# ruotianluo/ImageCaptioning.pytorch

Measured on NVIDIA H100. Metric: captions/sec at beam=5 seq_len=20, higher is better.
Workload: dtype f32 (fp32-grade: split-fp16 x3 tensor-core passes, fp32 accumulate)

## Files before the change

### imagecaptioning.pytorch_b200/_lib.py

```python
from __future__ import annotations

import ctypes
import os
from ctypes import POINTER, Structure, c_char_p, c_double, c_float, c_int, c_long, c_longlong, c_ulonglong, c_void_p

PKG = os.path.dirname(os.path.abspath(__file__))
LIB_PATH = os.path.join(PKG, 'libcapb200.so')

MODE_SIMT_FP32, MODE_TC_F16X3, MODE_TC_F16X1 = 0, 1, 2
MODES = {'simt_fp32': MODE_SIMT_FP32, 'tc_f16x3': MODE_TC_F16X3, 'tc_f16x1': MODE_TC_F16X1}
OP_MODES = dict(MODES, skinny_tf32x3=3, skinny_fp32=4, tf32x3_tc=5, tf32x3_tc_dgrad=6, tf32x3_tc_wgrad=7)
FAMILY_UPDOWN, FAMILY_NEWFC, FAMILY_ATT2IN2 = 0, 1, 2
FAMILY_AOA = 3
ENSEMBLE_MAX_MEMBERS = 8
SAMPLE_GREEDY, SAMPLE_MULTINOMIAL, SAMPLE_FORCED, SAMPLE_TEACHER, SAMPLE_TOPK, SAMPLE_TOPP = 0, 1, 2, 3, 4, 5


class ModelCfg(Structure):
    _fields_ = [('family', c_int), ('vocab_size', c_int), ('input_encoding_size', c_int), ('rnn_size', c_int), ('att_hid_size', c_int),
                ('fc_feat_size', c_int), ('att_feat_size', c_int), ('seq_length', c_int), ('numeric_mode', c_int)]


WEIGHT_FIELDS = ['embed', 'fc_embed_w', 'fc_embed_b', 'att_embed_w', 'att_embed_b', 'ctx2att_w', 'ctx2att_b', 'logit_w', 'logit_b',
                 'att_lstm_w_ih', 'att_lstm_w_hh', 'att_lstm_b_ih', 'att_lstm_b_hh', 'lang_lstm_w_ih', 'lang_lstm_w_hh', 'lang_lstm_b_ih',
# ... 183 lines not shown
    'capb200_vocab_select': (c_int, [c_void_p, c_long, c_int, c_int, c_int, c_float, c_float, c_ulonglong, c_ulonglong, c_void_p, c_int, c_void_p,
                                     c_void_p, c_void_p]),
    'capb200_engine_create': (c_void_p, [POINTER(ModelCfg)]),
    'capb200_engine_destroy': (None, [c_void_p]),
    'capb200_engine_bind_weights': (c_int, [c_void_p, POINTER(Weights), c_void_p]),
    'capb200_decode_beam': (c_int, [c_void_p, c_void_p, c_void_p, c_void_p, c_int, c_int, POINTER(BeamOpts), c_void_p, c_void_p, c_void_p, c_void_p,
                                    c_void_p, c_void_p, c_void_p]),
    'capb200_beam_record_logprobs': (c_int, [c_void_p, c_int, c_int, c_void_p, c_void_p]),
    'capb200_decode_beam_diverse': (c_int, [c_void_p, c_void_p, c_void_p, c_void_p, c_int, c_int, POINTER(DiverseOpts), c_void_p, c_void_p, c_void_p,
                                            c_void_p, c_void_p, c_void_p, c_void_p]),
    'capb200_decode_sample': (c_int, [c_void_p, c_void_p, c_void_p, c_void_p, c_int, c_int, POINTER(SampleOpts), c_void_p, c_long, c_void_p, c_void_p,
                                      c_void_p, c_void_p]),
    'capb200_engine_launch_count': (c_long, [c_void_p]),
    'capb200_engine_set_profiling': (c_int, [c_void_p, c_int]),
    'capb200_engine_read_profile': (c_int, [c_void_p, c_int, c_void_p, c_void_p, c_void_p, c_int]),
    'capb200_tfm_create': (c_void_p, [POINTER(TfmCfg)]),
    'capb200_tfm_destroy': (None, [c_void_p]),
    'capb200_tfm_bind_weights': (c_int, [c_void_p, POINTER(TfmWeights), c_void_p]),
    'capb200_tfm_decode_beam': (c_int, [c_void_p, c_void_p, c_void_p, c_int, c_int, POINTER(BeamOpts), c_void_p, c_void_p, c_void_p, c_void_p, c_void_p,
                                        c_void_p, c_void_p]),
    'capb200_tfm_beam_record_logprobs': (c_int, [c_void_p, c_int, c_int, c_void_p, c_void_p]),
    'capb200_tfm_decode_sample': (c_int, [c_void_p, c_void_p, c_void_p, c_int, c_int, POINTER(SampleOpts), c_void_p, c_long, c_void_p, c_void_p, c_void_p,
                                          c_void_p]),
    'capb200_tfm_launch_count': (c_long, [c_void_p]),
    'capb200_aoa_create': (c_void_p, [POINTER(AoaCfg)]),
    'capb200_aoa_destroy': (None, [c_void_p]),
    'capb200_aoa_bind_weights': (c_int, [c_void_p, POINTER(AoaWeights), c_void_p]),
    'capb200_aoa_decode_beam': (c_int, [c_void_p, c_void_p, c_void_p, c_int, c_int, POINTER(BeamOpts), c_void_p, c_void_p, c_void_p, c_void_p, c_void_p,
                                        c_void_p, c_void_p]),
    'capb200_aoa_beam_record_logprobs': (c_int, [c_void_p, c_int, c_int, c_void_p, c_void_p]),
    'capb200_aoa_decode_beam_diverse': (c_int, [c_void_p, c_void_p, c_void_p, c_int, c_int, POINTER(DiverseOpts), c_void_p, c_void_p, c_void_p, c_void_p,
                                                c_void_p, c_void_p, c_void_p]),
    'capb200_aoa_decode_sample': (c_int, [c_void_p, c_void_p, c_void_p, c_int, c_int, POINTER(SampleOpts), c_void_p, c_long, c_void_p, c_void_p, c_void_p,
                                          c_void_p]),
    'capb200_aoa_scst_step': (c_int, [c_void_p, c_void_p, c_int, c_int, POINTER(AoaScstOpts), c_void_p, c_void_p, c_void_p, c_int, POINTER(AoaWeights),
                                      c_void_p, c_void_p, c_void_p, c_void_p, c_void_p, c_void_p]),
    'capb200_aoa_xe_step': (c_int, [c_void_p, c_void_p, c_int, c_int, POINTER(AoaXeOpts), c_void_p, c_void_p, c_int, POINTER(AoaWeights), c_void_p,
                                    c_void_p, c_void_p]),
    'capb200_aoa_launch_count': (c_long, [c_void_p]),
    'capb200_ensemble_create': (c_void_p, []),
    'capb200_ensemble_destroy': (None, [c_void_p]),
    'capb200_ensemble_decode_beam': (c_int, [c_void_p, c_void_p, c_int, c_void_p, c_void_p, c_void_p, c_int, c_int, POINTER(BeamOpts), c_void_p, c_void_p,
                                             c_void_p, c_void_p, c_void_p, c_void_p, c_void_p]),
    'capb200_ensemble_beam_record_logprobs': (c_int, [c_void_p, c_int, c_int, c_void_p, c_void_p]),
    'capb200_ensemble_decode_sample': (c_int, [c_void_p, c_void_p, c_int, c_void_p, c_void_p, c_void_p, c_int, c_int, POINTER(SampleOpts), c_void_p, c_long,
                                               c_void_p, c_void_p, c_void_p, c_void_p]),
    'capb200_ensemble_launch_count': (c_long, [c_void_p]),
    'capb200_updown_scst_step': (c_int, [c_void_p, c_void_p, c_void_p, c_int, c_int, POINTER(ScstOpts), c_void_p, c_void_p, c_void_p, c_int,
                                         POINTER(UpdownGrads), c_void_p, c_void_p, c_void_p, c_void_p, c_void_p, c_void_p]),
    'capb200_att2in2_scst_step': (c_int, [c_void_p, c_void_p, c_void_p, c_int, c_int, POINTER(ScstOpts), c_void_p, c_void_p, c_void_p, c_int,
                                          POINTER(Att2in2Grads), c_void_p, c_void_p, c_void_p, c_void_p, c_void_p, c_void_p]),
    'capb200_att2in2_xe_step': (c_int, [c_void_p, c_void_p, c_void_p, c_int, c_int, POINTER(XeOpts), c_void_p, c_void_p, c_int, POINTER(Att2in2Grads),
                                        c_void_p, c_void_p, c_void_p]),
    'capb200_newfc_scst_step': (c_int, [c_void_p, c_void_p, c_void_p, c_int, c_int, POINTER(ScstOpts), c_void_p, c_void_p, c_void_p, c_int,
                                        POINTER(NewfcGrads), c_void_p, c_void_p, c_void_p, c_void_p, c_void_p, c_void_p]),
    'capb200_newfc_xe_step': (c_int, [c_void_p, c_void_p, c_void_p, c_int, c_int, POINTER(XeOpts), c_void_p, c_void_p, c_int, POINTER(NewfcGrads),
                                      c_void_p, c_void_p, c_void_p]),
    'capb200_dropout_mask': (c_int, [c_void_p, c_long, c_ulonglong, c_int, c_int, c_float, c_void_p]),
    'capb200_tfm_xe_step': (c_int, [c_void_p, c_void_p, c_int, c_int, POINTER(TfmXeOpts), c_void_p, c_void_p, c_int, POINTER(TfmWeights), c_void_p, c_void_p,
                                    c_void_p]),
    'capb200_tfm_scst_step': (c_int, [c_void_p, c_void_p, c_int, c_int, POINTER(TfmScstOpts), c_void_p, c_void_p, c_void_p, c_int, POINTER(TfmWeights),
                                      c_void_p, c_void_p, c_void_p, c_void_p, c_void_p, c_void_p]),
    'capb200_tfm_set_grad_events': (c_int, [c_void_p, c_void_p, c_int]),
    'capb200_adam_chunk_elems': (c_int, []),
    'capb200_adam_step': (c_int, [c_void_p, c_void_p, c_void_p, c_int, c_double, c_double, c_double, c_double, c_double, c_long, c_double, c_int, c_void_p]),
    'capb200_engine_set_grad_events': (c_int, [c_void_p, c_void_p, c_int]),
    'capb200_aoa_set_grad_events': (c_int, [c_void_p, c_void_p, c_int]),
    'capb200_cider_table_create': (c_void_p, [c_void_p, c_void_p, c_long, c_double, c_void_p]),
    'capb200_cider_table_destroy': (None, [c_void_p]),
    'capb200_cider_corpus_table_create': (c_void_p, []),
    'capb200_cider_table_reserve': (c_int, [c_void_p, c_long, c_int]),
    'capb200_cider_table_is_corpus': (c_int, [c_void_p]),
    'capb200_cider_scores': (c_int, [c_void_p, c_void_p, c_int, c_int, c_int, c_void_p, c_void_p, c_int, c_void_p, c_void_p, c_void_p]),
    'capb200_bleu4_scores': (c_int, [c_void_p, c_int, c_void_p, c_int, c_int, c_void_p, c_void_p, c_int, c_void_p, c_void_p]),
    'capb200_weighted_reward': (c_int, [c_void_p, POINTER(RewardWeights), c_void_p, c_int, c_void_p, c_int, c_int, c_void_p, c_void_p, c_int, c_void_p,
                                        c_void_p, c_void_p, c_void_p]),
    'capb200_updown_xe_step': (c_int, [c_void_p, c_void_p, c_void_p, c_int, c_int, POINTER(XeOpts), c_void_p, c_void_p, c_int, c_void_p, c_void_p,
                                       c_void_p, c_void_p]),
    'capb200_self_critical_reward': (c_int, [c_void_p, c_void_p, c_int, c_void_p, c_int, c_int, c_void_p, c_void_p, c_int, c_void_p, c_void_p,
                                             c_void_p]),
    'capb200_reward_criterion_forward': (c_int, [c_void_p, c_void_p, c_void_p, c_int, c_int, c_int, c_void_p, c_void_p, c_void_p, c_void_p]),
    'capb200_reward_criterion_backward': (c_int, [c_void_p, c_void_p, c_int, c_int, c_int, c_void_p, c_float, c_void_p, c_void_p]),
    'capb200_decode_gemm': (c_int, [c_void_p, c_void_p, c_int, c_int, c_int, c_int, POINTER(GemmEpilogue), c_void_p, c_int, c_void_p]),
    'capb200_updown_xe_vjp': (c_int, [c_void_p, c_void_p, c_void_p, c_int, c_int, POINTER(XeOpts), POINTER(VjpOpts), c_void_p, c_int,
                                      POINTER(UpdownGrads), c_void_p, c_void_p]),
    'capb200_updown_scst_vjp': (c_int, [c_void_p, c_void_p, c_void_p, c_int, c_int, POINTER(ScstOpts), POINTER(VjpOpts), POINTER(UpdownGrads),
                                        c_void_p, c_void_p, c_void_p]),
    'capb200_att2in2_xe_vjp': (c_int, [c_void_p, c_void_p, c_void_p, c_int, c_int, POINTER(XeOpts), POINTER(VjpOpts), c_void_p, c_int,
                                       POINTER(Att2in2Grads), c_void_p, c_void_p]),
    'capb200_att2in2_scst_vjp': (c_int, [c_void_p, c_void_p, c_void_p, c_int, c_int, POINTER(ScstOpts), POINTER(VjpOpts), POINTER(Att2in2Grads),
                                         c_void_p, c_void_p, c_void_p]),
    'capb200_newfc_xe_vjp': (c_int, [c_void_p, c_void_p, c_void_p, c_int, c_int, POINTER(XeOpts), POINTER(VjpOpts), c_void_p, c_int,
                                     POINTER(NewfcGrads), c_void_p, c_void_p]),
    'capb200_newfc_scst_vjp': (c_int, [c_void_p, c_void_p, c_void_p, c_int, c_int, POINTER(ScstOpts), POINTER(VjpOpts), POINTER(NewfcGrads),
                                       c_void_p, c_void_p, c_void_p]),
    'capb200_aoa_xe_vjp': (c_int, [c_void_p, c_void_p, c_int, c_int, POINTER(AoaXeOpts), POINTER(VjpOpts), c_void_p, c_int, POINTER(AoaWeights),
                                   c_void_p, c_void_p]),
    'capb200_aoa_scst_vjp': (c_int, [c_void_p, c_void_p, c_int, c_int, POINTER(AoaScstOpts), POINTER(VjpOpts), POINTER(AoaWeights), c_void_p,
                                     c_void_p, c_void_p]),
    'capb200_tfm_xe_vjp': (c_int, [c_void_p, c_void_p, c_int, c_int, POINTER(TfmXeOpts), POINTER(VjpOpts), c_void_p, c_int, POINTER(TfmWeights),
                                   c_void_p, c_void_p]),
    'capb200_tfm_scst_vjp': (c_int, [c_void_p, c_void_p, c_int, c_int, POINTER(TfmScstOpts), POINTER(VjpOpts), POINTER(TfmWeights), c_void_p,
                                     c_void_p, c_void_p]),
}

_lib = None


def load() -> ctypes.CDLL:
    global _lib
    if _lib is not None:
        return _lib
    if not os.path.exists(LIB_PATH):
        raise RuntimeError('capb200: %s is missing -- run `python imagecaptioning.pytorch_b200/build.py`; there is no CPU fallback' % LIB_PATH)
    lib = ctypes.CDLL(LIB_PATH)
    for name, (res, args) in SIGNATURES.items():
        fn = getattr(lib, name)
        fn.restype = res
        fn.argtypes = args
    if lib.capb200_abi_version() != 1:
        raise RuntimeError('capb200: ABI version mismatch')
    _lib = lib
    return lib


def check(rc: int, what: str = '') -> None:
    if rc != 0:
        msg = load().capb200_last_error()
        raise RuntimeError('capb200 %s failed: %s' % (what, msg.decode() if msg else 'unknown error'))


def ptr(t) -> int:
    if t is None:
        return None
    if hasattr(t, 'data_ptr'):
        return t.data_ptr()
    return t.ctypes.data


def current_stream() -> int:
    import torch
    return torch.cuda.current_stream().cuda_stream
```

### imagecaptioning.pytorch_b200/csrc/aoa_engine.cu

```cuda
#include <vector>

#include "../../include/capb200.h"
#include "common.cuh"
#include "engine_common.cuh"
#include "kernels.cuh"
#include "train_common.cuh"

using namespace capb200;

namespace capb200 {
__global__ void capb_add_vec_kernel(const float* a, const float* b, float* o, int n) {
    const int i = blockIdx.x * blockDim.x + threadIdx.x;
    if (i < n) o[i] = a[i] + b[i];
}
__global__ void capb_interleave_gates_kernel(const float* src, float* dst, int H) {
    const int i = blockIdx.x * blockDim.x + threadIdx.x;
    if (i < 4 * H) dst[i] = src[(i & 3) * H + (i >> 2)];
}
}

struct capb200_aoa_engine {
    capb200_aoa_cfg cfg{};
    capb200_aoa_weights w{};
    int V1 = 0, E = 0, H = 0, heads = 0, dk = 0, F = 0, T = 0, mode = 0;
// ... 11 lines not shown
    char* ws = nullptr;
    int capB = 0, capRows = 0, capR = 0, capBeam = 0;
    Planes in_att;
    Act rx, rln, rqkv, ratt, rt, att_e, mean, p_att_kv, g_mean;
    Act h0_in, h0_out, ctx_in, ctx_out, xt, gates, qln, qproj, att, t2;
    float* c0[2] = {nullptr, nullptr};
    long ld_c = 0;
    int core_cur = 0;
    DecodeBuffers d;
    std::vector<GemmTcPlan*> plans;
    char* tape = nullptr;
    size_t tape_bytes = 0;
    Tf32Context* tf32 = nullptr;
    cudaEvent_t grad_events[10] = {};
    cudaStream_t side = nullptr;
    cudaEvent_t ev_fork = nullptr, ev_join = nullptr;
    StepGraph sg;
};

namespace {

enum Site { A_ATT = 0, A_CTX, A_GMEAN, A_LSTM, A_Q, A_A2C, A_LOGIT, A_REF , A_COUNT = A_REF + 2 * CAPB200_AOA_REFINER_LAYERS };

void destroy_plans(capb200_aoa_engine* e) {
    for (auto& p : e->plans) { if (p) gemm_tc_plan_destroy(p); p = nullptr; }
}

int gemm(capb200_aoa_engine* e, int site, GemmProblem& g, int plan_rows, cudaStream_t st) {
    e->launches++;
    return run_gemm_mode(e->mode, &e->plans[site], g, plan_rows, st);
}

void layout_weights(capb200_aoa_engine* e, Arena& a) {
    const int H = e->H, E = e->E;
    for (int l = 0; l < CAPB200_AOA_REFINER_LAYERS; ++l) { e->r_qkv_w[l] = a.take<float>((long)3 * H * H); e->r_qkv_b[l] = a.take<float>(3 * H); }
    e->bsum = a.take<float>(4 * H);
    e->bsum_il = a.take<float>(4 * H);
    e->ld_xgate = round_up(4 * H, 8);
    e->xgate = a.take<float>((long)e->V1 * e->ld_xgate);
    if (!e->tc) return;
    e->p_att = carve_planes(a, H, e->F);
    e->p_ctx = carve_planes(a, 2 * H, H);
    e->p_logit = carve_planes(a, e->V1, H);
    e->p_ih_x = carve_planes(a, 4 * H, E);
    e->p_ih_c = carve_planes(a, 4 * H, H);
    e->p_hh = carve_planes(a, 4 * H, H);
    e->p_q = carve_planes(a, H, H);
    e->p_a2c_a = carve_planes(a, 2 * H, H);
    e->p_a2c_h = carve_planes(a, 2 * H, H);
    for (int l = 0; l < CAPB200_AOA_REFINER_LAYERS; ++l) {
        e->pr_qkv[l] = carve_planes(a, 3 * H, H);
        e->pr_aoa_a[l] = carve_planes(a, 2 * H, H);
        e->pr_aoa_q[l] = carve_planes(a, 2 * H, H);
    }
}

void layout_workspace(capb200_aoa_engine* e, Arena& a, int B, int rows, int R, int beam) {
    const int H = e->H, E = e->E, T = e->T;
    const bool tc = e->tc;
    const long BR = (long)B * R;
    if (tc) e->in_att = carve_planes(a, BR, e->F);
    e->rx.carve(a, BR, H, false);
    e->rln.carve(a, BR, H, tc);
    e->rqkv.carve(a, BR, 3 * H, false);
    e->ratt.carve(a, BR, H, tc);
    e->rt.carve(a, BR, 2 * H, false);
    e->att_e.carve(a, BR, H, tc);
    e->mean.carve(a, B, H, tc);
    e->p_att_kv.carve(a, BR, 2 * H, false);
    e->g_mean.carve(a, B, 4 * H, false);
    e->h0_in.carve(a, rows, H, tc);
    e->h0_out.carve(a, rows, H, tc);
    e->ctx_in.carve(a, rows, H, tc);
    e->ctx_out.carve(a, rows, H, tc);
    e->xt.carve(a, rows, E, tc);
    e->gates.carve(a, rows, 4 * H, false);
    e->qln.carve(a, rows, H, tc);
    e->qproj.carve(a, rows, H, false);
    e->att.carve(a, rows, H, tc);
    e->t2.carve(a, rows, 2 * H, false);
    e->ld_c = round_up(H, 8);
    for (int i = 0; i < 2; ++i) e->c0[i] = a.take<float>((long)rows * e->ld_c);
    e->d.carve(a, B, rows, beam, T);
}

int ensure_workspace(capb200_aoa_engine* e, int B, int rows, int R, int beam, cudaStream_t st) {
    if (B <= e->capB && rows <= e->capRows && R <= e->capR && beam <= e->capBeam && e->ws != nullptr) return 0;
    const int nB = B > e->capB ? B : e->capB, nRows = rows > e->capRows ? rows : e->capRows;
    const int nR = R > e->capR ? R : e->capR, nBeam = beam > e->capBeam ? beam : e->capBeam;
    Arena dry;
    layout_workspace(e, dry, nB, nRows, nR, nBeam);
    const size_t need = dry.off + 256;
    CAPB_CHECK_CUDA(cudaStreamSynchronize(st));
    destroy_plans(e);
    if (e->ws) CAPB_CHECK_CUDA(cudaFree(e->ws));
    e->ws = nullptr;
    CAPB_CHECK_CUDA(cudaMalloc(&e->ws, need));
    Arena real;
    real.base = e->ws;
    layout_workspace(e, real, nB, nRows, nR, nBeam);
    e->capB = nB; e->capRows = nRows; e->capR = nR; e->capBeam = nBeam;
    CAPB_CHECK_CUDA(cudaMemsetAsync(e->ws, 0, need, st));
    return fill_int_launch(e->d.neg1, nRows, -1, st);
}

int pack(capb200_aoa_engine* e, const float* w, long ldw, int rows, int cols, const Planes& p, cudaStream_t st) {
    e->launches++;
    return split_planes_launch(w, ldw, rows, cols, p.hi, p.lo, p.ld, st);
}
int pack_gates(capb200_aoa_engine* e, const float* w, long ldw, int H, int cols, const Planes& p, cudaStream_t st) {
    e->launches++;
    return split_planes_interleave_launch(w, ldw, H, cols, p.hi, p.lo, p.ld, st);
}

int prepare(capb200_aoa_engine* e, const float* att, const float* mask, int B, int R, cudaStream_t st) {
    CAPB_NVTX("capb200 aoa prepare_feature (att_embed, refiner, ctx2att)");
    const int H = e->H, E = e->E, BR = B * R, capBR = e->capB * e->capR;
    const capb200_aoa_weights& w = e->w;
    ActView in; in.f = const_cast<float*>(att); in.ld = e->F;
    if (e->tc) {
        e->launches++;
        if (split_planes_launch(att, e->F, BR, e->F, e->in_att.hi, e->in_att.lo, e->in_att.ld, st)) return 1;
        in.hi = e->in_att.hi; in.lo = e->in_att.lo;
    }
    {
        GemmProblem g;
        g.M = BR; g.N = H; g.nseg = 1;
        g.seg[0] = seg_of(in, w.att_embed_w, e->F, e->p_att, e->F);
        g.seg[0].lda_h = e->in_att.ld;
        g.epi.bias = w.att_embed_b; g.epi.relu = 1;
        g.epi.C = e->rx.v.f; g.epi.ldc = e->rx.v.ld;
        if (gemm(e, A_ATT, g, capBR, st)) return 1;
    }
    if (mask != nullptr) { e->launches++; if (mask_rows_launch(e->rx.v, B, R, H, mask, R, st)) return 1; }
    for (int l = 0; l < CAPB200_AOA_REFINER_LAYERS; ++l) {
        const capb200_aoa_refiner_layer& L = w.refiner[l];
        e->launches++;
        if (layer_norm_launch(BR, H, e->rx.v.f, e->rx.v.ld, L.ln_a, L.ln_b, 1e-6f, e->rln.v, st)) return 1;
        {
            GemmProblem g;
            g.M = BR; g.N = 3 * H; g.nseg = 1;
            g.seg[0] = seg_of(e->rln.v, e->r_qkv_w[l], H, e->pr_qkv[l], H);
            g.epi.bias = e->r_qkv_b[l];
            g.epi.C = e->rqkv.v.f; g.epi.ldc = e->rqkv.v.ld;
            if (gemm(e, A_REF + 2 * l, g, capBR, st)) return 1;
        }
        e->launches++;
        if (enc_self_attention_launch(B, R, e->heads, e->dk, e->rqkv.v.f, e->rqkv.v.f + H, e->rqkv.v.f + 2 * H, e->rqkv.v.ld, mask, R, e->ratt.v, st)) return 1;
        {
            GemmProblem g;
            g.M = BR; g.N = 2 * H; g.nseg = 2;
            g.seg[0] = seg_of(e->ratt.v, L.aoa_w, 2 * H, e->pr_aoa_a[l], H);
            g.seg[1] = seg_of(e->rln.v, L.aoa_w + H, 2 * H, e->pr_aoa_q[l], H);
            g.epi.bias = L.aoa_b;
            g.epi.C = e->rt.v.f; g.epi.ldc = e->rt.v.ld;
            if (gemm(e, A_REF + 2 * l + 1, g, capBR, st)) return 1;
        }
        e->launches++;
        ActView xo = e->rx.v;
        if (glu_launch(BR, H, e->rt.v.f, e->rt.v.ld, e->rx.v.f, e->rx.v.ld, xo, st)) return 1;
    }
    e->launches++;
    if (layer_norm_launch(BR, H, e->rx.v.f, e->rx.v.ld, w.refiner_norm_a, w.refiner_norm_b, 1e-6f, e->att_e.v, st)) return 1;
    e->launches++;
    if (masked_mean_launch(B, R, H, e->att_e.v.f, e->att_e.v.ld, mask, R, e->mean.v, st)) return 1;
    {
        GemmProblem g;
        g.M = BR; g.N = 2 * H; g.nseg = 1;
        g.seg[0] = seg_of(e->att_e.v, w.ctx2att_w, H, e->p_ctx, H);
        g.epi.bias = w.ctx2att_b;
        g.epi.C = e->p_att_kv.v.f; g.epi.ldc = e->p_att_kv.v.ld;
        if (gemm(e, A_CTX, g, capBR, st)) return 1;
    }
    {
        GemmProblem g;
        g.M = B; g.N = 4 * H; g.nseg = 1;
        g.seg[0] = seg_of(e->mean.v, w.att_lstm_w_ih + E, E + H, e->p_ih_c, H);
        g.epi.bias = e->tc ? e->bsum_il : e->bsum;
        g.epi.C = e->g_mean.v.f; g.epi.ldc = e->g_mean.v.ld;
        if (gemm(e, A_GMEAN, g, e->capB, st)) return 1;
    }
    return 0;
}

int core_step(capb200_aoa_engine* e, int rows, int rpi, const int* tokens, const int* src_row, float* logits, long ld_logits, int B, int R,
              const float* mask, cudaStream_t st) {
    const int H = e->H, E = e->E;
    const capb200_aoa_weights& w = e->w;
    StateCopy s0, s1;
    s0.src = e->h0_out.v.f; s0.ld_src = e->h0_out.v.ld; s0.dst = e->h0_in.v;
    s1.src = e->ctx_out.v.f; s1.ld_src = e->ctx_out.v.ld; s1.dst = e->ctx_in.v;
    e->launches++;
    if (state_gather_embed_launch(rows, tokens, src_row, w.embed, E, 0, 1, e->xt.v, H, 2, s0, s1, st)) return 1;
    const int cur = e->core_cur, nxt = cur ^ 1;
    {
        GemmProblem g;
        g.M = rows; g.N = 4 * H; g.nseg = 2;
        g.seg[0] = seg_of(e->ctx_in.v, w.att_lstm_w_ih + E, E + H, e->p_ih_c, H);
        g.seg[1] = seg_of(e->h0_in.v, w.att_lstm_w_hh, H, e->p_hh, H);
        g.epi.row_bias = e->g_mean.v.f; g.epi.ld_row_bias = e->g_mean.v.ld; g.epi.rows_per_group = rpi;
        if (e->tc) {
            g.epi.lstm = 1; g.epi.H = H;
            g.epi.c_prev = e->c0[cur]; g.epi.ld_cprev = e->ld_c; g.epi.src_row = src_row;
            g.epi.c_out = e->c0[nxt]; g.epi.ld_cout = e->ld_c;
            g.epi.gather_bias = e->xgate; g.epi.ld_gb = e->ld_xgate; g.epi.gather_idx = tokens;
            g.epi.h_f = e->h0_out.v.f; g.epi.h_hi = e->h0_out.v.hi; g.epi.h_lo = e->h0_out.v.lo; g.epi.ld_h = e->h0_out.v.ld;
        } else {
            g.epi.C = e->gates.v.f; g.epi.ldc = e->gates.v.ld;
        }
        if (gemm(e, A_LSTM, g, e->capRows, st)) return 1;
    }
    if (!e->tc) {
        e->launches++;
        if (lstm_pointwise_launch(rows, H, e->gates.v.f, e->gates.v.ld, src_row, e->c0[cur], e->ld_c, e->c0[nxt], e->ld_c, e->h0_out.v, e->xgate,
                                  e->ld_xgate, tokens, st)) return 1;
    }
    e->core_cur = nxt;
    e->launches++;
    if (layer_norm_launch(rows, H, e->h0_out.v.f, e->h0_out.v.ld, w.attn_norm_a, w.attn_norm_b, 1e-6f, e->qln.v, st)) return 1;
    {
        GemmProblem g;
        g.M = rows; g.N = H; g.nseg = 1;
        g.seg[0] = seg_of(e->qln.v, w.attn_q_w, H, e->p_q, H);
        g.epi.bias = w.attn_q_b;
        g.epi.C = e->qproj.v.f; g.epi.ldc = e->qproj.v.ld;
        if (gemm(e, A_Q, g, e->capRows, st)) return 1;
    }
    e->launches++;
    if (cross_attention_launch(rows, rpi, e->heads, e->dk, R, e->qproj.v.f, e->qproj.v.ld, e->p_att_kv.v.f + H, e->p_att_kv.v.f, e->p_att_kv.v.ld, mask, R,
                               e->att.v, st)) return 1;
    {
        GemmProblem g;
        g.M = rows; g.N = 2 * H; g.nseg = 2;
        g.seg[0] = seg_of(e->att.v, w.att2ctx_w, 2 * H, e->p_a2c_a, H);
        g.seg[1] = seg_of(e->h0_out.v, w.att2ctx_w + H, 2 * H, e->p_a2c_h, H);
        g.epi.bias = w.att2ctx_b;
        g.epi.C = e->t2.v.f; g.epi.ldc = e->t2.v.ld;
        if (gemm(e, A_A2C, g, e->capRows, st)) return 1;
    }
    e->launches++;
    if (glu_launch(rows, H, e->t2.v.f, e->t2.v.ld, nullptr, 0, e->ctx_out.v, st)) return 1;
    GemmProblem g;
    g.M = rows; g.N = e->V1; g.nseg = 1;
    g.seg[0] = seg_of(e->ctx_out.v, w.logit_w, H, e->p_logit, H);
    g.epi.bias = w.logit_b;
    g.epi.C = logits; g.epi.ldc = ld_logits;
    (void)B;
    return gemm(e, A_LOGIT, g, e->capRows, st);
}

int check_ready(capb200_aoa_engine* e) {
    CAPB_REQUIRE(e != nullptr, "null engine");
    CAPB_REQUIRE(e->bound, "capb200_aoa_bind_weights has not been called");
    CAPB_CHECK_RANGE();
    return 0;
}

}

namespace capb200 {

int aoa_member_info(capb200_aoa_engine* e, MemberInfo* m) {
    if (check_ready(e)) return 1;
    m->family = CAPB200_FAMILY_AOA;
    m->V1 = e->V1; m->T = e->T;
    m->attends = true;
    m->graph_ok = true;
    m->ws = e->ws; m->wblock = e->wblock;
    m->fresh = e->d.neg1;
    m->launches = &e->launches;
    return 0;
}

int aoa_decode_workspace(capb200_aoa_engine* e, int B, int rows, int R, int beam, cudaStream_t st) {
    return ensure_workspace(e, B, rows, R, beam, st);
}

int aoa_decode_prepare(capb200_aoa_engine* e, const float* att, const float* mask, int B, int R, cudaStream_t st) {
    if (prepare(e, att, mask, B, R, st)) return 1;
    e->core_cur = 0;
    return 0;
}

int aoa_decode_core(capb200_aoa_engine* e, int rows, int rpi, const int* tokens, const int* src_row, float* logits, long ld, int R,
                    const float* mask, cudaStream_t st) {
    return core_step(e, rows, rpi, tokens, src_row, logits, ld, 0, R, mask, st);
}

}

extern "C" {

capb200_aoa_engine* capb200_aoa_create(const capb200_aoa_cfg* c) {
    if (c == nullptr) { set_error("null cfg"); return nullptr; }
    if (c->heads < 1 || c->rnn_size % c->heads != 0) { set_error("rnn_size must be divisible by the head count"); return nullptr; }
    if (c->numeric_mode < 0 || c->numeric_mode > 2) { set_error("unknown numeric mode"); return nullptr; }
    if (c->seq_length < 1 || c->seq_length > 64) { set_error("seq_length must be in 1..64"); return nullptr; }
    int ndev = 0;
    if (cudaGetDeviceCount(&ndev) != cudaSuccess || ndev == 0) { set_error("no CUDA device: the capb200 engine has no CPU fallback"); return nullptr; }
    capb200_aoa_engine* e = new capb200_aoa_engine();
    e->cfg = *c;
    e->V1 = c->vocab_size + 1; e->E = c->input_encoding_size; e->H = c->rnn_size; e->heads = c->heads; e->dk = c->rnn_size / c->heads;
    e->F = c->att_feat_size; e->T = c->seq_length; e->mode = c->numeric_mode;
    e->tc = c->numeric_mode != CAPB200_MODE_SIMT_FP32;
    e->plans.assign(A_COUNT, nullptr);
    return e;
}

void capb200_aoa_destroy(capb200_aoa_engine* e) {
    if (e == nullptr) return;
    destroy_plans(e);
    cudaFree(e->wblock);
    cudaFree(e->ws);
    e->d.release();
    cudaFree(e->tape);
    e->sg.destroy();
    tf32_context_destroy(e->tf32);
    if (e->ev_fork) cudaEventDestroy(e->ev_fork);
    if (e->ev_join) cudaEventDestroy(e->ev_join);
    if (e->side) cudaStreamDestroy(e->side);
    delete e;
}

long capb200_aoa_launch_count(const capb200_aoa_engine* e) { return e ? e->launches : 0; }

int capb200_aoa_bind_weights(capb200_aoa_engine* e, const capb200_aoa_weights* w, void* stream) {
    CAPB_REQUIRE(e != nullptr && w != nullptr, "null argument");
    cudaStream_t st = static_cast<cudaStream_t>(stream);
    CAPB_REQUIRE(w->embed && w->att_embed_w && w->ctx2att_w && w->att_lstm_w_ih && w->att_lstm_w_hh && w->attn_q_w && w->att2ctx_w && w->logit_w,
// ... 429 lines not shown
```

### imagecaptioning.pytorch_b200/csrc/common.cuh

```cuda
#pragma once
#include <atomic>
#include <cstdint>
#include <cstdio>
#include <cstring>
#include <string>
#include <cuda.h>
#include <cuda_fp16.h>
#include <cuda_runtime.h>

namespace capb200 {

void set_error(const std::string& msg);
#define CAPB_CHECK_CUDA(expr)                                                                          \
    do {                                                                                               \
        cudaError_t _e = (expr);                                                                       \
        if (_e != cudaSuccess) {                                                                       \
            capb200::set_error(std::string(#expr) + " failed: " + cudaGetErrorString(_e) + " at " +    \
                               __FILE__ + ":" + std::to_string(__LINE__));                            \
            return 1;                                                                                  \
        }                                                                                              \
    } while (0)
#define CAPB_REQUIRE(cond, msg)                                                                        \
    do {                                                                                               \
        if (!(cond)) {                                                                                 \
            capb200::set_error(std::string("requirement failed: ") + #cond + " -- " + (msg));          \
            return 1;                                                                                  \
        }                                                                                              \
    } while (0)

inline int cdiv(int a, int b) { return (a + b - 1) / b; }
inline long round_up(long a, long b) { return (a + b - 1) / b * b; }

inline bool first_use_on_device(std::atomic<unsigned long long>& mask) {
    int dev = 0;
    if (cudaGetDevice(&dev) != cudaSuccess || dev < 0 || dev > 63) return true;
    const unsigned long long bit = 1ull << dev;
    return (mask.fetch_or(bit) & bit) == 0;
}

inline int sm_count() {
    static std::atomic<int> cache[64];
    int dev = 0;
    if (cudaGetDevice(&dev) != cudaSuccess || dev < 0 || dev > 63) dev = 0;
    int n = cache[dev].load();
    if (n == 0) {
        if (cudaDeviceGetAttribute(&n, cudaDevAttrMultiProcessorCount, dev) != cudaSuccess || n < 1) n = 132;
        cache[dev].store(n);
    }
    return n;
}

__device__ __forceinline__ void split_f32(float x, __half& hi, __half& lo) {
    hi = __float2half_rn(x);
    lo = __float2half_rn(x - __half2float(hi));
}

constexpr int kMaxSeg = 3;
struct GemmSeg {
    const float* A = nullptr;
    long lda = 0;
    const float* W = nullptr;
    long ldw = 0;
    const __half* A_hi = nullptr;
    const __half* A_lo = nullptr;
    long lda_h = 0;
    const __half* W_hi = nullptr;
    const __half* W_lo = nullptr;
    long ldw_h = 0;
    int K = 0;
};
struct GemmEpilogue {
    const float* bias = nullptr;
    const float* row_bias = nullptr;
    long ld_row_bias = 0;
    int rows_per_group = 1;
    const float* residual = nullptr;
    long ld_res = 0;
    int relu = 0;
    float* C = nullptr;
    long ldc = 0;
    __half* C_hi = nullptr;
    __half* C_lo = nullptr;
    long ldcs = 0;
    int lstm = 0;
    int H = 0;
    const float* c_prev = nullptr;
    long ld_cprev = 0;
    const int* src_row = nullptr;
    float* c_out = nullptr;
    long ld_cout = 0;
    const float* gather_bias = nullptr;
    long ld_gb = 0;
    const int* gather_idx = nullptr;
    float* h_f = nullptr;
    __half* h_hi = nullptr;
    __half* h_lo = nullptr;
    long ld_h = 0;
    unsigned long long* trace = nullptr;
};

__device__ __forceinline__ float fast_sigmoid(float x) { return __fdividef(1.0f, 1.0f + __expf(-x)); }
__device__ __forceinline__ float fast_tanh(float x) {
    const float e = __expf(2.0f * x);
    return 1.0f - __fdividef(2.0f, 1.0f + e);
}
__device__ __forceinline__ void fast_tanh4(const float (&x)[4], float (&t)[4]) {
    float y[4];
#pragma unroll
    for (int i = 0; i < 4; ++i) y[i] = 1.0f + __expf(fminf(2.0f * x[i], 20.0f));
    const float p01 = y[0] * y[1], p23 = y[2] * y[3];
    const float r = __fdividef(1.0f, p01 * p23);
    const float r01 = r * p23, r23 = r * p01;
    t[0] = fmaf(-2.0f, r01 * y[1], 1.0f);
    t[1] = fmaf(-2.0f, r01 * y[0], 1.0f);
    t[2] = fmaf(-2.0f, r23 * y[3], 1.0f);
    t[3] = fmaf(-2.0f, r23 * y[2], 1.0f);
}
struct GemmProblem {
    int M = 0, N = 0, nseg = 0;
    GemmSeg seg[kMaxSeg];
    GemmEpilogue epi;
};

enum NumericMode : int {
    kModeSimtFp32 = 0,
    kModeTcF16x3 = 1,
    kModeTcF16x1 = 2,
};

int gemm_simt_launch(const GemmProblem& p, cudaStream_t stream);

struct GemmTcPlan;
GemmTcPlan* gemm_tc_plan_create(const GemmProblem& p, int passes);
int gemm_tc_tile_n(int M, int N);
int gemm_tc_tile_m(int M, int N, int bn);
void gemm_tc_plan_destroy(GemmTcPlan* plan);
int gemm_tc_plan_launch(GemmTcPlan* plan, const GemmEpilogue* epi_override, int M_override, cudaStream_t stream);
bool gemm_tc_supported(const GemmProblem& p, std::string* why);

int split_planes_launch(const float* x, long ldx, int rows, int cols, __half* hi, __half* lo, long ldh, cudaStream_t stream);
int* range_flag_ptr();
int range_flag_read(int reset);
#define CAPB_CHECK_RANGE()                                                                                              \
    do {                                                                                                                \
        if (capb200::range_flag_read(0)) {                                                                              \
            capb200::set_error("a value with |x| >= 65504 (or inf/nan) reached a split-fp16 conversion in an earlier call: results of the "   \
                               "tensor-core modes are invalid for such inputs/weights (DESIGN.md section 3); capb200_range_status(1) clears the flag"); \
            return 1;                                                                                                   \
        }                                                                                                               \
    } while (0)
int split_planes_interleave_launch(const float* x, long ldx, int H, int cols, __half* hi, __half* lo, long ldh, cudaStream_t stream);

}
```

### imagecaptioning.pytorch_b200/csrc/engine.cu

```cuda
#include <map>
#include <mutex>
#include <vector>

#include "../../include/capb200.h"
#include "common.cuh"
#include "kernels.cuh"
#include "engine_common.cuh"
#include "train_common.cuh"

namespace capb200 {

static thread_local std::string g_last_error;
void set_error(const std::string& msg) { g_last_error = msg; }
const char* last_error_cstr() { return g_last_error.c_str(); }

__global__ void capb_fill_int_kernel(int* p, int n, int v) {
    const int i = blockIdx.x * blockDim.x + threadIdx.x;
    if (i < n) p[i] = v;
}
__global__ void capb_load_token_column_kernel(const long long* src, long ld, int col, int n, int* dst) {
    const int i = blockIdx.x * blockDim.x + threadIdx.x;
    if (i < n) dst[i] = (int)src[(long)i * ld + col];
}
__global__ void capb_store_token_column_kernel(const int* src, int n, long long* dst, long ld, int col) {
// ... 104 lines not shown
}

void layout_weights(capb200_engine* e, Arena& a) {
    const int H = e->H, E = e->E, A = e->A, V1 = e->V1;
    const bool updown = e->cfg.family == CAPB200_FAMILY_UPDOWN;
    e->bsum_att = a.take<float>(4 * H);
    e->bsum_lang = a.take<float>(4 * H);
    e->bsum_core = a.take<float>(5 * H);
    e->bsum_att_il = a.take<float>(4 * H);
    e->bsum_lang_il = a.take<float>(4 * H);
    if (updown) { e->ld_xgate = round_up(4 * H, 8); e->xgate = a.take<float>((long)V1 * e->ld_xgate); }
    if (!e->tc) return;
    e->p_logit = carve_planes(a, V1, H);
    if (updown) {
        e->p_fc = carve_planes(a, H, e->cfg.fc_feat_size);
        e->p_attw = carve_planes(a, H, e->cfg.att_feat_size);
        e->p_ctx = carve_planes(a, A, H);
        e->p_a_ih_h = carve_planes(a, 4 * H, H);
        e->p_a_ih_fc = carve_planes(a, 4 * H, H);
        e->p_a_ih_x = carve_planes(a, 4 * H, E);
        e->p_a_hh = carve_planes(a, 4 * H, H);
        e->p_l_ih_a = carve_planes(a, 4 * H, H);
        e->p_l_ih_h = carve_planes(a, 4 * H, H);
        e->p_l_hh = carve_planes(a, 4 * H, H);
        e->p_h2att = carve_planes(a, A, H);
    } else if (e->cfg.family == CAPB200_FAMILY_ATT2IN2) {
        e->p_attw = carve_planes(a, H, e->cfg.att_feat_size);
        e->p_ctx = carve_planes(a, A, H);
        e->p_h2att = carve_planes(a, A, H);
        e->p_i2h = carve_planes(a, 5 * H, E);
        e->p_h2h = carve_planes(a, 5 * H, H);
        e->p_a2c = carve_planes(a, 2 * H, H);
    } else {
        e->p_fc = carve_planes(a, E, e->cfg.fc_feat_size);
        e->p_i2h = carve_planes(a, 5 * H, E);
        e->p_h2h = carve_planes(a, 5 * H, H);
    }
}

bool attends(const capb200_engine* e) { return e->cfg.family != CAPB200_FAMILY_NEWFC; }

int pack(capb200_engine* e, const float* w, long ldw, int rows, int cols, const Planes& p, cudaStream_t st) {
    e->launches++;
    return split_planes_launch(w, ldw, rows, cols, p.hi, p.lo, p.ld, st);
}
int pack_gates(capb200_engine* e, const float* w, long ldw, int H, int cols, const Planes& p, cudaStream_t st) {
    e->launches++;
    return split_planes_interleave_launch(w, ldw, H, cols, p.hi, p.lo, p.ld, st);
}

void layout_workspace(capb200_engine* e, Arena& a, int B, int rows, int R, int beam) {
    const int H = e->H, E = e->E, A = e->A, T = e->T;
    const bool updown = e->cfg.family == CAPB200_FAMILY_UPDOWN;
    const bool attn = attends(e);
    const bool tc = e->tc;
    if (tc) {
        e->in_fc = carve_planes(a, B, e->cfg.fc_feat_size);
        if (attn) e->in_att = carve_planes(a, (long)B * R, e->cfg.att_feat_size);
    }
    e->fc_e.carve(a, B, updown ? H : E, tc);
    if (attn) {
        e->att_e.carve(a, (long)B * R, H, tc);
        e->p_att.carve(a, (long)B * R, A, false);
        e->att_res.carve(a, rows, H, tc);
        e->att_h.carve(a, rows, A, false);
    }
    if (updown) {
        e->g_fc.carve(a, B, 4 * H, false);
        e->h1_in.carve(a, rows, H, tc);
        e->h1_out.carve(a, rows, H, tc);
    }
    e->xt.carve(a, rows, E, tc);
    e->h0_in.carve(a, rows, H, tc);
    e->h0_out.carve(a, rows, H, tc);
    e->gates.carve(a, rows, 5 * H, false);
    e->ld_c = round_up(H, 8);
    for (int i = 0; i < 2; ++i) {
        e->c0[i] = a.take<float>((long)rows * e->ld_c);
        e->c1[i] = a.take<float>((long)rows * e->ld_c);
    }
    e->img_of_row = a.take<int>(rows);
    e->att_score = a.take<float>((long)rows * (R > 0 ? R : 1));
    e->d.carve(a, B, rows, beam, T);
}

int ensure_workspace(capb200_engine* e, int B, int rows, int R, int beam, cudaStream_t st) {
    if (B <= e->capB && rows <= e->capRows && R <= e->capR && beam <= e->capBeam && e->ws != nullptr) return 0;
    const int nB = B > e->capB ? B : e->capB, nRows = rows > e->capRows ? rows : e->capRows;
    const int nR = R > e->capR ? R : e->capR, nBeam = beam > e->capBeam ? beam : e->capBeam;
    Arena dry;
    layout_workspace(e, dry, nB, nRows, nR, nBeam);
    const size_t need = dry.off + 256;
    CAPB_CHECK_CUDA(cudaStreamSynchronize(st));
    destroy_plans(e);
    if (e->ws) CAPB_CHECK_CUDA(cudaFree(e->ws));
    e->ws = nullptr;
    CAPB_CHECK_CUDA(cudaMalloc(&e->ws, need));
    e->ws_bytes = need;
    Arena real;
    real.base = e->ws;
    layout_workspace(e, real, nB, nRows, nR, nBeam);
    e->capB = nB; e->capRows = nRows; e->capR = nR; e->capBeam = nBeam;
    CAPB_CHECK_CUDA(cudaMemsetAsync(e->ws, 0, need, st));
    return fill_int_launch(e->d.neg1, nRows, -1, st);
}

int run_gemm_inner(capb200_engine* e, int id, GemmProblem& g, int plan_rows, cudaStream_t st) {
    e->launches++;
    if (!e->tc) return gemm_simt_launch(g, st);
    if (e->plans[id] == nullptr) {
        GemmProblem planned = g;
        planned.M = plan_rows;
        e->plans[id] = gemm_tc_plan_create(planned, e->mode == CAPB200_MODE_TC_F16X3 ? 3 : 1);
        if (e->plans[id] == nullptr) return 1;
    }
    return gemm_tc_plan_launch(e->plans[id], &g.epi, g.M, st);
}

int run_gemm(capb200_engine* e, int id, GemmProblem& g, int plan_rows, cudaStream_t st) {
    if (!e->profiling) return run_gemm_inner(e, id, g, plan_rows, st);
    if (e->ev_used + 2 > e->ev_pool.size()) {
        for (int i = 0; i < 64; ++i) {
            cudaEvent_t ev;
            CAPB_CHECK_CUDA(cudaEventCreate(&ev));
            e->ev_pool.push_back(ev);
        }
    }
    double k_total = 0;
    for (int s = 0; s < g.nseg; ++s) k_total += g.seg[s].K;
    CAPB_CHECK_CUDA(cudaEventRecord(e->ev_pool[e->ev_used], st));
    const int rc = run_gemm_inner(e, id, g, plan_rows, st);
    CAPB_CHECK_CUDA(cudaEventRecord(e->ev_pool[e->ev_used + 1], st));
    e->ev_used += 2;
    e->ev_ids.push_back(id);
    e->ev_flops.push_back(2.0 * g.M * g.N * k_total);
    return rc;
}

int prepare(capb200_engine* e, const float* fc, const float* att, const float* mask, int B, int R, cudaStream_t st) {
    CAPB_NVTX("capb200 prepare_feature (fc_embed, att_embed, ctx2att)");
    const int H = e->H, E = e->E, A = e->A;
    const bool updown = e->cfg.family == CAPB200_FAMILY_UPDOWN;
    const capb200_weights& w = e->w;
    ActView fc_in;  fc_in.f = const_cast<float*>(fc);  fc_in.ld = e->cfg.fc_feat_size;
    if (e->tc && e->cfg.family != CAPB200_FAMILY_ATT2IN2) {
        e->launches++;
        if (split_planes_launch(fc, e->cfg.fc_feat_size, B, e->cfg.fc_feat_size, e->in_fc.hi, e->in_fc.lo, e->in_fc.ld, st)) return 1;
    }
    if (e->cfg.family != CAPB200_FAMILY_ATT2IN2) {
        GemmProblem g;
        g.M = B; g.N = updown ? H : E; g.nseg = 1;
        g.seg[0] = seg_of(fc_in, w.fc_embed_w, e->cfg.fc_feat_size, e->p_fc, e->cfg.fc_feat_size);
        g.seg[0].A_hi = e->in_fc.hi; g.seg[0].A_lo = e->in_fc.lo; g.seg[0].lda_h = e->in_fc.ld;
        g.epi.bias = w.fc_embed_b; g.epi.relu = updown ? 1 : 0;
        g.epi.C = e->fc_e.v.f; g.epi.ldc = e->fc_e.v.ld; g.epi.C_hi = e->fc_e.v.hi; g.epi.C_lo = e->fc_e.v.lo; g.epi.ldcs = e->fc_e.v.ld;
        if (run_gemm(e, G_FC, g, e->capB, st)) return 1;
    }
    if (!attends(e)) return 0;
    ActView att_in; att_in.f = const_cast<float*>(att); att_in.ld = e->cfg.att_feat_size;
    if (e->tc) {
        e->launches++;
        if (split_planes_launch(att, e->cfg.att_feat_size, B * R, e->cfg.att_feat_size, e->in_att.hi, e->in_att.lo, e->in_att.ld, st)) return 1;
    }
    {
        GemmProblem g;
        g.M = B * R; g.N = H; g.nseg = 1;
// ... 24 lines not shown
        g.epi.C = e->g_fc.v.f; g.epi.ldc = e->g_fc.v.ld;
        if (run_gemm(e, G_GFC, g, e->capB, st)) return 1;
    }
    return 0;
}

int core_step(capb200_engine* e, int rows, int rpi, const int* tokens, const int* src_row, float* logits, long ld_logits, int n_images, int R,
              const float* mask, cudaStream_t st) {
    const int H = e->H, E = e->E, A = e->A, V1 = e->V1;
    const capb200_weights& w = e->w;
    if (e->cfg.family == CAPB200_FAMILY_UPDOWN) {
        StateCopy s0, s1;
        s0.src = e->h0_out.v.f; s0.ld_src = e->h0_out.v.ld; s0.dst = e->h0_in.v;
        s1.src = e->h1_out.v.f; s1.ld_src = e->h1_out.v.ld; s1.dst = e->h1_in.v;
        const bool xg = e->use_xgate;
        e->launches++;
        if (state_gather_embed_launch(rows, tokens, src_row, w.embed, E, xg ? 0 : E, 1, e->xt.v, H, 2, s0, s1, st)) return 1;
        const int cur = e->core_cur, nxt = cur ^ 1;
        {
            GemmProblem g;
            g.M = rows; g.N = 4 * H;
            g.seg[0] = seg_of(e->h1_in.v, w.att_lstm_w_ih, E + 2 * H, e->p_a_ih_h, H);
            g.seg[1] = seg_of(e->h0_in.v, w.att_lstm_w_hh, H, e->p_a_hh, H);
            g.nseg = 2;
            if (!xg) { g.seg[2] = seg_of(e->xt.v, w.att_lstm_w_ih + 2 * H, E + 2 * H, e->p_a_ih_x, E); g.nseg = 3; }
            g.epi.row_bias = e->g_fc.v.f; g.epi.ld_row_bias = e->g_fc.v.ld; g.epi.rows_per_group = rpi;
            if (e->tc) {
                g.epi.lstm = 1; g.epi.H = H;
                g.epi.c_prev = e->c0[cur]; g.epi.ld_cprev = e->ld_c; g.epi.src_row = src_row;
                g.epi.c_out = e->c0[nxt]; g.epi.ld_cout = e->ld_c;
                g.epi.gather_bias = xg ? e->xgate : nullptr; g.epi.ld_gb = e->ld_xgate; g.epi.gather_idx = tokens;
                g.epi.h_f = e->h0_out.v.f; g.epi.h_hi = e->h0_out.v.hi; g.epi.h_lo = e->h0_out.v.lo; g.epi.ld_h = e->h0_out.v.ld;
            } else {
                g.epi.C = e->gates.v.f; g.epi.ldc = e->gates.v.ld;
            }
            if (run_gemm(e, G_LSTM1, g, e->capRows, st)) return 1;
        }
        if (!e->tc) {
            e->launches++;
            if (lstm_pointwise_launch(rows, H, e->gates.v.f, e->gates.v.ld, src_row, e->c0[cur], e->ld_c, e->c0[nxt], e->ld_c, e->h0_out.v,
                                      xg ? e->xgate : nullptr, e->ld_xgate, tokens, st)) return 1;
        }
        {
            GemmProblem g;
            g.M = rows; g.N = A; g.nseg = 1;
            g.seg[0] = seg_of(e->h0_out.v, w.h2att_w, H, e->p_h2att, H);
            g.epi.bias = w.h2att_b;
            g.epi.C = e->att_h.v.f; g.epi.ldc = e->att_h.v.ld;
            if (run_gemm(e, G_H2ATT, g, e->capRows, st)) return 1;
        }
        e->launches += 2;
        if (additive_attention_launch(n_images, rpi, R, A, H, e->att_h.v.f, e->att_h.v.ld, e->p_att.v.f, e->p_att.v.ld, e->att_e.v.f, e->att_e.v.ld,
                                      mask, R, w.alpha_w, w.alpha_b, e->att_score, e->att_res.v, st)) return 1;
        {
            GemmProblem g;
            g.M = rows; g.N = 4 * H; g.nseg = 3;
            g.seg[0] = seg_of(e->att_res.v, w.lang_lstm_w_ih, 2 * H, e->p_l_ih_a, H);
            g.seg[1] = seg_of(e->h0_out.v, w.lang_lstm_w_ih + H, 2 * H, e->p_l_ih_h, H);
            g.seg[2] = seg_of(e->h1_in.v, w.lang_lstm_w_hh, H, e->p_l_hh, H);
            if (e->tc) {
                g.epi.bias = e->bsum_lang_il;
                g.epi.lstm = 1; g.epi.H = H;
                g.epi.c_prev = e->c1[cur]; g.epi.ld_cprev = e->ld_c; g.epi.src_row = src_row;
                g.epi.c_out = e->c1[nxt]; g.epi.ld_cout = e->ld_c;
                g.epi.h_f = e->h1_out.v.f; g.epi.h_hi = e->h1_out.v.hi; g.epi.h_lo = e->h1_out.v.lo; g.epi.ld_h = e->h1_out.v.ld;
            } else {
                g.epi.bias = e->bsum_lang;
                g.epi.C = e->gates.v.f; g.epi.ldc = e->gates.v.ld;
            }
            if (run_gemm(e, G_LSTM2, g, e->capRows, st)) return 1;
        }
        if (!e->tc) {
            e->launches++;
            if (lstm_pointwise_launch(rows, H, e->gates.v.f, e->gates.v.ld, src_row, e->c1[cur], e->ld_c, e->c1[nxt], e->ld_c, e->h1_out.v,
                                      nullptr, 0, nullptr, st)) return 1;
        }
        e->core_cur = nxt;
        {
            GemmProblem g;
            g.M = rows; g.N = V1; g.nseg = 1;
            g.seg[0] = seg_of(e->h1_out.v, w.logit_w, H, e->p_logit, H);
            g.epi.bias = w.logit_b;
            g.epi.C = logits; g.epi.ldc = ld_logits;
            if (run_gemm(e, G_LOGIT, g, e->capRows, st)) return 1;
        }
        return 0;
    }
    if (e->cfg.family == CAPB200_FAMILY_ATT2IN2) {
        StateCopy s0, s1;
        s0.src = e->h0_out.v.f; s0.ld_src = e->h0_out.v.ld; s0.dst = e->h0_in.v;
        e->launches++;
        if (state_gather_embed_launch(rows, tokens, src_row, w.embed, E, E, 1, e->xt.v, H, 1, s0, s1, st)) return 1;
        const int cur = e->core_cur, nxt = cur ^ 1;
        {
            GemmProblem g;
            g.M = rows; g.N = A; g.nseg = 1;
            g.seg[0] = seg_of(e->h0_in.v, w.h2att_w, H, e->p_h2att, H);
            g.epi.bias = w.h2att_b;
            g.epi.C = e->att_h.v.f; g.epi.ldc = e->att_h.v.ld;
            if (run_gemm(e, G_H2ATT, g, e->capRows, st)) return 1;
        }
        e->launches += 2;
        if (additive_attention_launch(n_images, rpi, R, A, H, e->att_h.v.f, e->att_h.v.ld, e->p_att.v.f, e->p_att.v.ld, e->att_e.v.f, e->att_e.v.ld,
                                      mask, R, w.alpha_w, w.alpha_b, e->att_score, e->att_res.v, st)) return 1;
        {
            GemmProblem g;
            g.M = rows; g.N = 5 * H; g.nseg = 2;
            g.seg[0] = seg_of(e->xt.v, w.i2h_w, E, e->p_i2h, E);
            g.seg[1] = seg_of(e->h0_in.v, w.h2h_w, H, e->p_h2h, H);
            g.epi.bias = e->bsum_core;
            g.epi.C = e->gates.v.f; g.epi.ldc = e->gates.v.ld;
            if (run_gemm(e, G_CORE, g, e->capRows, st)) return 1;
        }
        {
            GemmProblem g;
            g.M = rows; g.N = 2 * H; g.nseg = 1;
            g.seg[0] = seg_of(e->att_res.v, w.a2c_w, H, e->p_a2c, H);
            g.epi.residual = e->gates.v.f + 3 * H; g.epi.ld_res = e->gates.v.ld;
            g.epi.C = e->gates.v.f + 3 * H; g.epi.ldc = e->gates.v.ld;
            if (run_gemm(e, G_A2C, g, e->capRows, st)) return 1;
        }
        e->launches++;
        if (maxout_pointwise_launch(rows, H, e->gates.v.f, e->gates.v.ld, src_row, e->c0[cur], e->ld_c, e->c0[nxt], e->ld_c, e->h0_out.v, st)) return 1;
        e->core_cur = nxt;
        GemmProblem g;
        g.M = rows; g.N = V1; g.nseg = 1;
        g.seg[0] = seg_of(e->h0_out.v, w.logit_w, H, e->p_logit, H);
        g.epi.bias = w.logit_b;
        g.epi.C = logits; g.epi.ldc = ld_logits;
        return run_gemm(e, G_LOGIT, g, e->capRows, st);
    }
    const bool fresh = (src_row == e->d.neg1);
    for (int pass = fresh ? 0 : 1; pass < 2; ++pass) {
        StateCopy s0, s1;
        s0.src = e->h0_out.v.f; s0.ld_src = e->h0_out.v.ld; s0.dst = e->h0_in.v;
        const int* srcs = (pass == 0) ? e->d.neg1 : (fresh ? nullptr : src_row);
        e->launches++;
        if (pass == 0) {
            if (state_gather_embed_launch(rows, e->img_of_row, srcs, e->fc_e.v.f, e->fc_e.v.ld, E, 0, e->xt.v, H, 1, s0, s1, st)) return 1;
        } else {
            if (state_gather_embed_launch(rows, tokens, srcs, w.embed, E, E, 0, e->xt.v, H, 1, s0, s1, st)) return 1;
        }
        const int cur = e->core_cur, nxt = cur ^ 1;
        GemmProblem g;
        g.M = rows; g.N = 5 * H; g.nseg = 2;
        g.seg[0] = seg_of(e->xt.v, w.i2h_w, E, e->p_i2h, E);
        g.seg[1] = seg_of(e->h0_in.v, w.h2h_w, H, e->p_h2h, H);
        g.epi.bias = e->bsum_core;
        g.epi.C = e->gates.v.f; g.epi.ldc = e->gates.v.ld;
        if (run_gemm(e, G_CORE, g, e->capRows, st)) return 1;
        e->launches++;
        if (maxout_pointwise_launch(rows, H, e->gates.v.f, e->gates.v.ld, srcs, e->c0[cur], e->ld_c, e->c0[nxt], e->ld_c, e->h0_out.v, st)) return 1;
        e->core_cur = nxt;
    }
    GemmProblem g;
    g.M = rows; g.N = V1; g.nseg = 1;
    g.seg[0] = seg_of(e->h0_out.v, w.logit_w, H, e->p_logit, H);
    g.epi.bias = w.logit_b;
    g.epi.C = logits; g.epi.ldc = ld_logits;
    return run_gemm(e, G_LOGIT, g, e->capRows, st);
}

int check_ready(capb200_engine* e) {
    CAPB_REQUIRE(e != nullptr, "null engine");
    CAPB_REQUIRE(e->bound, "capb200_engine_bind_weights has not been called");
    CAPB_CHECK_RANGE();
    return 0;
}

}

namespace capb200 {

int lstm_member_info(capb200_engine* e, MemberInfo* m) {
    if (check_ready(e)) return 1;
    m->family = e->cfg.family;
    m->V1 = e->V1; m->T = e->T;
    m->attends = attends(e);
    m->graph_ok = !e->profiling;
    m->ws = e->ws; m->wblock = e->wblock;
    m->fresh = e->d.neg1;
    m->launches = &e->launches;
    return 0;
}

int lstm_decode_workspace(capb200_engine* e, int B, int rows, int R, int beam, int rows_per_image, cudaStream_t st) {
    if (ensure_workspace(e, B, rows, R, beam, st)) return 1;
    if (!attends(e)) { iota_div_kernel<<<cdiv(rows, 256), 256, 0, st>>>(e->img_of_row, rows, rows_per_image); e->launches++; }
    return 0;
}

int lstm_decode_prepare(capb200_engine* e, const float* fc, const float* att, const float* mask, int B, int R, cudaStream_t st) {
    if (prepare(e, fc, att, mask, B, R, st)) return 1;
    e->core_cur = 0;
    return 0;
}

int lstm_decode_core(capb200_engine* e, int rows, int rpi, const int* tokens, const int* src_row, float* logits, long ld, int B, int R,
                     const float* mask, cudaStream_t st) {
    return core_step(e, rows, rpi, tokens, src_row, logits, ld, B, R, mask, st);
}

}

extern "C" {

const char* capb200_last_error(void) { return g_last_error.c_str(); }
int capb200_abi_version(void) { return CAPB200_ABI_VERSION; }
int capb200_range_status(int reset) { return range_flag_read(reset); }

capb200_engine* capb200_engine_create(const capb200_model_cfg* cfg) {
    if (cfg == nullptr) { set_error("null cfg"); return nullptr; }
    if (cfg->family != CAPB200_FAMILY_UPDOWN && cfg->family != CAPB200_FAMILY_NEWFC && cfg->family != CAPB200_FAMILY_ATT2IN2) {
        set_error("unknown model family");
        return nullptr;
    }
    if (cfg->numeric_mode < 0 || cfg->numeric_mode > 2) { set_error("unknown numeric mode"); return nullptr; }
    if (cfg->seq_length < 1 || cfg->seq_length > 64) { set_error("seq_length must be in 1..64"); return nullptr; }
    int ndev = 0;
    if (cudaGetDeviceCount(&ndev) != cudaSuccess || ndev == 0) {
        set_error("no CUDA device: the capb200 engine has no CPU fallback");
        return nullptr;
    }
    capb200_engine* e = new capb200_engine();
    e->cfg = *cfg;
    e->V1 = cfg->vocab_size + 1;
    e->E = cfg->input_encoding_size;
    e->H = cfg->rnn_size;
    e->A = cfg->att_hid_size;
    e->T = cfg->seq_length;
    e->mode = cfg->numeric_mode;
    e->tc = cfg->numeric_mode != CAPB200_MODE_SIMT_FP32;
    return e;
}

void capb200_engine_destroy(capb200_engine* e) {
    if (e == nullptr) return;
    destroy_plans(e);
    for (cudaEvent_t ev : e->ev_pool) cudaEventDestroy(ev);
    cudaFree(e->wblock);
    cudaFree(e->ws);
    e->d.release();
// ... 324 lines not shown
    g.seg[0].A = x; g.seg[0].lda = K; g.seg[0].W = w; g.seg[0].ldw = K; g.seg[0].K = K;
    g.epi.bias = b; g.epi.C = y; g.epi.ldc = N;
    const long ldh = round_up(K, 64);
    __half* scratch = nullptr;
    GemmTcPlan* plan = nullptr;
    int rc = 0;
    if (mode != CAPB200_MODE_SIMT_FP32) {
        CAPB_CHECK_CUDA(cudaMalloc(&scratch, (size_t)(M + N) * ldh * 2 * sizeof(__half)));
        __half* xh = scratch; __half* xl = xh + (size_t)M * ldh;
        __half* wh = xl + (size_t)M * ldh; __half* wl = wh + (size_t)N * ldh;
        rc = split_planes_launch(x, K, M, K, xh, xl, ldh, st) | split_planes_launch(w, K, N, K, wh, wl, ldh, st);
        g.seg[0].A_hi = xh; g.seg[0].A_lo = xl; g.seg[0].lda_h = ldh;
        g.seg[0].W_hi = wh; g.seg[0].W_lo = wl; g.seg[0].ldw_h = ldh;
        plan = rc ? nullptr : gemm_tc_plan_create(g, mode == CAPB200_MODE_TC_F16X3 ? 3 : 1);
        if (plan == nullptr) rc = 1;
    }
    cudaEvent_t e0, e1;
    cudaEventCreate(&e0);
    cudaEventCreate(&e1);
    for (int i = 0; i < 3 + iters && !rc; ++i) {
        if (i == 3) cudaEventRecord(e0, st);
        rc = plan ? gemm_tc_plan_launch(plan, nullptr, 0, st) : gemm_simt_launch(g, st);
    }
    cudaEventRecord(e1, st);
    if (cudaStreamSynchronize(st) != cudaSuccess) { set_error(std::string("bench_linear: ") + cudaGetErrorString(cudaGetLastError())); rc = 1; }
    float ms = 0.f;
    if (!rc) { cudaEventElapsedTime(&ms, e0, e1); *ms_per_launch = ms / iters; }
    cudaEventDestroy(e0);
    cudaEventDestroy(e1);
    if (plan) gemm_tc_plan_destroy(plan);
    if (scratch) cudaFree(scratch);
    return rc;
}

int capb200_decode_gemm(const float* x, const float* w, int M, int N, int K, int mode, const capb200_gemm_epilogue* epi, unsigned long long* trace_host,
                        int n_slots, void* stream) {
    cudaStream_t st = static_cast<cudaStream_t>(stream);
    CAPB_REQUIRE(x && w && epi && M > 0 && N > 0 && K > 0, "bad argument");
    CAPB_REQUIRE(mode == CAPB200_MODE_TC_F16X3 || mode == CAPB200_MODE_TC_F16X1, "the decode GEMM runs in the tc_f16x3 / tc_f16x1 modes");
    CAPB_REQUIRE(trace_host == nullptr || (n_slots >= 296 * 16 && mode == CAPB200_MODE_TC_F16X3), "the trace needs 296 x 16 slots and tc_f16x3");
    GemmProblem g;
    g.M = M; g.N = N; g.nseg = 1;
    g.seg[0].K = K;
    GemmEpilogue& e = g.epi;
    e.bias = epi->bias; e.row_bias = epi->row_bias; e.ld_row_bias = epi->ld_row_bias; e.rows_per_group = epi->rows_per_group;
    e.residual = epi->residual; e.ld_res = epi->ld_res; e.relu = epi->relu;
    e.C = epi->C; e.ldc = epi->ldc;
    e.C_hi = reinterpret_cast<__half*>(epi->C_hi); e.C_lo = reinterpret_cast<__half*>(epi->C_lo); e.ldcs = epi->ldcs;
    e.lstm = epi->lstm; e.H = epi->H;
    e.c_prev = epi->c_prev; e.ld_cprev = epi->ld_cprev; e.src_row = epi->src_row;
    e.c_out = epi->c_out; e.ld_cout = epi->ld_cout;
    e.gather_bias = epi->gather_bias; e.ld_gb = epi->ld_gb; e.gather_idx = epi->gather_idx;
    e.h_f = epi->h_f; e.h_hi = reinterpret_cast<__half*>(epi->h_hi); e.h_lo = reinterpret_cast<__half*>(epi->h_lo); e.ld_h = epi->ld_h;
    CAPB_REQUIRE(e.C_hi == nullptr || e.C_lo != nullptr, "C_hi needs C_lo");
    CAPB_REQUIRE(e.h_hi == nullptr || e.h_lo != nullptr, "h_hi needs h_lo");
    CAPB_REQUIRE(e.row_bias == nullptr || e.rows_per_group >= 1, "rows_per_group must be >= 1");
    CAPB_REQUIRE(e.gather_bias == nullptr || e.gather_idx != nullptr, "gather_bias needs gather_idx");
    const long ldh = round_up(K, 64);
    __half* scratch = nullptr;
    unsigned long long* trace = nullptr;
    CAPB_CHECK_CUDA(cudaMalloc(&scratch, (size_t)(M + N) * ldh * 2 * sizeof(__half)));
    if (trace_host != nullptr) {
        CAPB_CHECK_CUDA(cudaMalloc(&trace, sizeof(unsigned long long) * 296 * 16));
        CAPB_CHECK_CUDA(cudaMemsetAsync(trace, 0, sizeof(unsigned long long) * 296 * 16, st));
    }
    __half* xh = scratch; __half* xl = xh + (size_t)M * ldh;
    __half* wh = xl + (size_t)M * ldh; __half* wl = wh + (size_t)N * ldh;
    int rc = split_planes_launch(x, K, M, K, xh, xl, ldh, st) | split_planes_launch(w, K, N, K, wh, wl, ldh, st);
    g.seg[0].A_hi = xh; g.seg[0].A_lo = xl; g.seg[0].lda_h = ldh;
    g.seg[0].W_hi = wh; g.seg[0].W_lo = wl; g.seg[0].ldw_h = ldh;
    GemmTcPlan* plan = rc ? nullptr : gemm_tc_plan_create(g, mode == CAPB200_MODE_TC_F16X3 ? 3 : 1);
    if (plan == nullptr) rc = 1;
    for (int i = 0; i < (trace ? 3 : 1) && !rc; ++i) rc = gemm_tc_plan_launch(plan, nullptr, 0, st);
    if (!rc && trace) {
        GemmEpilogue ep = g.epi;
        ep.trace = trace;
        rc = gemm_tc_plan_launch(plan, &ep, 0, st);
    }
    if (cudaStreamSynchronize(st) != cudaSuccess) { set_error(std::string("decode_gemm: ") + cudaGetErrorString(cudaGetLastError())); rc = 1; }
    if (!rc && trace) CAPB_CHECK_CUDA(cudaMemcpy(trace_host, trace, sizeof(unsigned long long) * 296 * 16, cudaMemcpyDeviceToHost));
    if (plan) gemm_tc_plan_destroy(plan);
    cudaFree(scratch);
    if (trace) cudaFree(trace);
    return rc;
}

int capb200_gemm_tile_n(int M, int N) { return gemm_tc_tile_n(M, N); }

int capb200_gemm_tile_m(int M, int N) { return gemm_tc_tile_m(M, N, gemm_tc_tile_n(M, N)); }

int capb200_lstm_cell(const float* x, int Kx, const float* h, const float* c, const float* w_ih, const float* w_hh, const float* b_ih,
                      const float* b_hh, float* h_out, float* c_out, int M, int H, int mode, void* stream) {
    cudaStream_t st = static_cast<cudaStream_t>(stream);
    CAPB_REQUIRE(x && h && c && w_ih && w_hh && b_ih && b_hh && h_out && c_out, "null argument");
    float* gates = nullptr;
    CAPB_CHECK_CUDA(cudaMallocAsync(&gates, sizeof(float) * ((size_t)M * 4 * H + 4 * H), st));
    float* bsum = gates + (size_t)M * 4 * H;
    add_vec_kernel<<<cdiv(4 * H, 256), 256, 0, st>>>(b_ih, b_hh, bsum, 4 * H);
    int rc = capb200_linear(x, Kx, w_ih, Kx, bsum, gates, 4 * H, M, 4 * H, Kx, 0, mode, stream);
    float* g2 = nullptr;
    if (!rc) {
        CAPB_CHECK_CUDA(cudaMallocAsync(&g2, sizeof(float) * (size_t)M * 4 * H, st));
        rc = capb200_linear(h, H, w_hh, H, nullptr, g2, 4 * H, M, 4 * H, H, 0, mode, stream);
        if (!rc) add_vec_kernel<<<cdiv(M * 4 * H, 256), 256, 0, st>>>(gates, g2, gates, M * 4 * H);
    }
    if (!rc) {
        ActView ho; ho.f = h_out; ho.ld = H;
        rc = lstm_pointwise_launch(M, H, gates, 4 * H, nullptr, c, H, c_out, H, ho, nullptr, 0, nullptr, st);
    }
    if (g2) cudaFreeAsync(g2, st);
    cudaFreeAsync(gates, st);
    return rc;
}

int capb200_additive_attention(const float* att_h, const float* p_att, const float* att, const float* mask, const float* alpha_w,
                               const float* alpha_b, float* out, int n_images, int rows_per_image, int R, int A, int H, void* stream) {
    CAPB_REQUIRE(att_h && p_att && att && alpha_w && alpha_b && out, "null argument");
    ActView o; o.f = out; o.ld = H;
    cudaStream_t st = static_cast<cudaStream_t>(stream);
    float* scratch = nullptr;
    CAPB_CHECK_CUDA(cudaMallocAsync(&scratch, sizeof(float) * (size_t)n_images * rows_per_image * R, st));
    const int rc = additive_attention_launch(n_images, rows_per_image, R, A, H, att_h, A, p_att, A, att, H, mask, R, alpha_w, alpha_b, scratch, o, st);
    cudaFreeAsync(scratch, st);
    return rc;
}

int capb200_log_softmax_topk(float* logits, long ld, int rows, int V1, int twice, int k, float* top_val, int* top_idx, void* stream) {
    CAPB_REQUIRE(logits != nullptr && rows > 0 && V1 > 0, "bad argument");
    VocabStepArgs va;
    va.rows = rows; va.V1 = V1; va.logits = logits; va.ld = ld; va.twice = twice; va.topk = k; va.top_val = top_val; va.top_idx = top_idx;
    return vocab_step_launch(va, static_cast<cudaStream_t>(stream));
}

int capb200_vocab_stats_topk(const float* logits, long ld, int rows, int V1, int twice, int k, float* stats, float* top_val, int* top_idx, void* stream) {
    CAPB_REQUIRE(logits != nullptr && stats != nullptr && top_val != nullptr && top_idx != nullptr, "null argument");
    CAPB_REQUIRE(rows > 0 && V1 > 0 && ld >= V1 && k > 0, "bad argument");
    CAPB_REQUIRE((reinterpret_cast<uintptr_t>(stats) & 7) == 0, "stats must be 8-byte aligned");
    VocabStepArgs va;
    va.rows = rows; va.V1 = V1; va.logits = const_cast<float*>(logits); va.ld = ld; va.twice = twice;
    va.topk = k; va.top_val = top_val; va.top_idx = top_idx;
    va.stats = reinterpret_cast<float2*>(stats);
    return vocab_step_launch(va, static_cast<cudaStream_t>(stream));
}

int capb200_vocab_select(float* logits, long ld, int rows, int V1, int select, float top, float temperature, unsigned long long seed,
                         unsigned long long step, int* unfinished, int first_step, int* tokens_out, float* picked_lp, void* stream) {
    CAPB_REQUIRE(logits != nullptr && tokens_out != nullptr && picked_lp != nullptr, "null argument");
    CAPB_REQUIRE(rows > 0 && V1 > 0 && ld >= V1, "bad argument");
    CAPB_REQUIRE(select == 1 || select == 2 || select == 4 || select == 5, "select must be 1 (greedy), 2 (multinomial), 4 (top-k) or 5 (nucleus)");
    CAPB_REQUIRE(temperature > 0.f, "temperature must be positive");
    CAPB_REQUIRE(select != 4 || top >= 1.f, "top-k sampling needs k >= 1");
    CAPB_REQUIRE(select != 5 || (top > 0.f && top <= 1.f), "nucleus sampling needs 0 < p <= 1");
    VocabStepArgs va;
    va.rows = rows; va.V1 = V1; va.logits = logits; va.ld = ld;
    va.select = select; va.top = top; va.temperature = temperature; va.seed = seed; va.step = step;
    va.unfinished = unfinished; va.first_step = first_step; va.tokens_out = tokens_out; va.picked_lp = picked_lp;
    return vocab_step_launch(va, static_cast<cudaStream_t>(stream));
}

}

namespace {

struct Tape : StepTape {
    int* tok;
    float *xt, *g1, *h0, *c0, *atth, *alpha, *attres, *g2, *h1, *c1, *out;
// ... 679 lines not shown
```

### imagecaptioning.pytorch_b200/csrc/engine_common.cuh

```cuda
#pragma once
#include <cstdio>
#include <cstdlib>
#include <cstring>

#include "../../include/capb200.h"
#include "common.cuh"
#include "kernels.cuh"
#include "nvtx.cuh"

struct capb200_cider_table {
    capb200::CiderTable* t = nullptr;
};

namespace capb200 {

struct Planes {
    __half* hi = nullptr;
    __half* lo = nullptr;
    long ld = 0;
};

struct Arena {
    char* base = nullptr;
    size_t off = 0;
    template <typename T>
    T* take(size_t n) {
        off = (off + 255) & ~size_t(255);
        T* p = base ? reinterpret_cast<T*>(base + off) : nullptr;
        off += n * sizeof(T);
        return p;
    }
};

struct Act {
    ActView v;
    void carve(Arena& a, long rows, long cols, bool planes) {
        v.ld = round_up(cols, 64);
        v.f = a.take<float>(rows * v.ld);
        if (planes) {
            v.hi = a.take<__half>(rows * v.ld);
            v.lo = a.take<__half>(rows * v.ld);
        } else {
            v.hi = v.lo = nullptr;
        }
    }
};

inline DecodeEdits to_edits(const capb200_decode_edits& c) {
    DecodeEdits e;
    e.constraint = c.decoding_constraint;
    e.unk_col = c.unk_col;
    e.n_bad = (c.bad_endings != nullptr && c.n_bad_endings > 0) ? c.n_bad_endings : 0;
    e.bad = c.bad_endings;
    e.trigrams = c.block_trigrams;
    e.trigram_rows = c.trigram_rows;
    return e;
}

inline Planes carve_planes(Arena& a, long rows, long cols) {
    Planes p;
    p.ld = round_up(cols, 64);
    p.hi = a.take<__half>(rows * p.ld);
    p.lo = a.take<__half>(rows * p.ld);
    return p;
}


inline GemmSeg seg_of(const ActView& a, const float* w, long ldw, const Planes& wp, int K) {
    GemmSeg s;
    s.A = a.f; s.lda = a.ld; s.W = w; s.ldw = ldw;
    s.A_hi = a.hi; s.A_lo = a.lo; s.lda_h = a.ld;
    s.W_hi = wp.hi; s.W_lo = wp.lo; s.ldw_h = wp.ld;
    s.K = K;
    return s;
}


inline int run_gemm_mode(int mode, GemmTcPlan** plan, GemmProblem& g, int plan_rows, cudaStream_t st) {
    if (mode == 0) return gemm_simt_launch(g, st);
    if (*plan == nullptr) {
        GemmProblem planned = g;
        planned.M = plan_rows;
        *plan = gemm_tc_plan_create(planned, mode == 1 ? 3 : 1);
        if (*plan == nullptr) return 1;
    }
    return gemm_tc_plan_launch(*plan, &g.epi, g.M, st);
}


struct DecodeBuffers {
    int *tokens = nullptr, *src_row = nullptr, *neg1 = nullptr, *unfinished = nullptr, *forced = nullptr;
    float* top_val = nullptr;
    int* top_idx = nullptr;
    float* top_val_e = nullptr;
    int* top_idx_e = nullptr;
    float2* slab_stats = nullptr;
    BeamState bs;
    long long* rec_seq = nullptr;
    int *rec_len = nullptr, *rec_hist = nullptr, *out_hist = nullptr, *tmp_len = nullptr;
    float *rec_p = nullptr, *rec_raw = nullptr, *tmp_p = nullptr, *tmp_raw = nullptr;
    float* slab = nullptr;
    size_t slab_bytes = 0;
    float2* dbs_stats = nullptr;
    size_t dbs_stats_bytes = 0;
    int* dbs_done_cnt = nullptr;
    size_t dbs_done_bytes = 0;
    const float2* last_stats = nullptr;
    long slab_step_stride = 0;
    int last_B = 0, last_beam = 0;
    DecodeEdits last_edits;
    cudaGraphExec_t loop_exec = nullptr;
    unsigned long long loop_key[8] = {0, 0, 0, 0, 0, 0, 0, 0}, seen_key[8] = {0, 0, 0, 0, 0, 0, 0, 0};
    long loop_launches = 0;
    bool graph_broken = false;

    void release() {
        if (loop_exec) cudaGraphExecDestroy(loop_exec);
        loop_exec = nullptr;
        cudaFree(slab);
        cudaFree(dbs_stats);
        cudaFree(dbs_done_cnt);
        slab = nullptr; dbs_stats = nullptr; dbs_done_cnt = nullptr;
    }

    void carve(Arena& a, int B, int rows, int beam, int T) {
        tokens = a.take<int>(rows);
        src_row = a.take<int>(rows);
        neg1 = a.take<int>(rows);
        unfinished = a.take<int>(rows);
        forced = a.take<int>(rows);
        top_val = a.take<float>((long)rows * 16);
        top_idx = a.take<int>((long)rows * 16);
        top_val_e = a.take<float>((long)rows * 16);
        top_idx_e = a.take<int>((long)rows * 16);
        slab_stats = a.take<float2>((long)rows * T);
        const long rec = (long)B * beam * T;
        bs.sums = a.take<float>((long)B * beam);
        bs.seq_a = a.take<int>(rec);
        bs.seq_b = a.take<int>(rec);
        bs.hist_a = a.take<int>(rec);
        bs.hist_b = a.take<int>(rec);
        bs.done_cnt = a.take<int>(B);
        bs.done_seq = a.take<int>(rec * T);
        bs.done_hist = a.take<int>(rec * T);
        bs.done_len = a.take<int>(rec);
        bs.done_p = a.take<double>(rec);
        bs.done_raw = a.take<float>(rec);
        bs.tokens = tokens;
        bs.src_row = src_row;
        rec_seq = a.take<long long>(rec);
        rec_hist = a.take<int>(rec);
        out_hist = a.take<int>(rec);
        rec_len = a.take<int>((long)B * beam);
        rec_p = a.take<float>((long)B * beam);
        rec_raw = a.take<float>((long)B * beam);
        tmp_len = a.take<int>((long)B * beam);
        tmp_p = a.take<float>((long)B * beam);
        tmp_raw = a.take<float>((long)B * beam);
    }
};

__global__ void capb_fill_int_kernel(int* p, int n, int v);
__global__ void capb_load_token_column_kernel(const long long* src, long ld, int col, int n, int* dst);
int fill_int_launch(int* p, int n, int v, cudaStream_t st);
int load_token_column_launch(const long long* src, long ld, int col, int n, int* dst, cudaStream_t st);
int store_token_column_launch(const int* src, int n, long long* dst, long ld, int col, cudaStream_t st);

inline const int* beam_ancestors(const BeamState& s, int t) { return ((t - 1) & 1) ? s.hist_a : s.hist_b; }

inline unsigned long long loop_graph_key(const void* ws, const void* wblock, const void* mask, int R, int family) {
    unsigned long long h = 1469598103934665603ull;
    auto mix = [&](unsigned long long v) { h ^= v; h *= 1099511628211ull; };
    mix(reinterpret_cast<uintptr_t>(ws)); mix(reinterpret_cast<uintptr_t>(wblock)); mix(reinterpret_cast<uintptr_t>(mask));
    mix((unsigned long long)R); mix((unsigned long long)family + 17);
    return h | 1ull;
}

inline int grow_buffer(void** p, size_t* bytes, size_t need, cudaStream_t st) {
    if (need <= *bytes) return 0;
    CAPB_CHECK_CUDA(cudaStreamSynchronize(st));
    if (*p) CAPB_CHECK_CUDA(cudaFree(*p));
    *p = nullptr;
    *bytes = 0;
    const cudaError_t e = cudaMalloc(p, need);
    if (e != cudaSuccess) {
        (void)cudaGetLastError();
        *p = nullptr;
        set_error("cannot allocate " + std::to_string(need >> 20) + " MB of device workspace (" + cudaGetErrorString(e) +
                  "); its size grows with batch, length and V + 1: DESIGN.md, 'Vocabularies above 51 199 words'");
        return 1;
    }
    *bytes = need;
    return 0;
}

template <class Loop>
int run_beam_loop(DecodeBuffers& d, const unsigned long long (&key)[8], bool use_graph, long* launches, cudaStream_t st, Loop run_loop) {
    static const bool graphs_off = getenv("CAPB200_NO_GRAPH") != nullptr;
    const bool debug = getenv("CAPB200_GRAPH_DEBUG") != nullptr;
    const bool try_graph = use_graph && !graphs_off && !d.graph_broken;
    if (try_graph && d.loop_exec != nullptr && memcmp(key, d.loop_key, sizeof(key)) == 0) {
        CAPB_CHECK_CUDA(cudaGraphLaunch(d.loop_exec, st));
        *launches += d.loop_launches;
        if (debug) fprintf(stderr, "capb200: beam loop replayed from its CUDA graph\n");
    } else if (try_graph && memcmp(key, d.seen_key, sizeof(key)) == 0) {
        if (d.loop_exec != nullptr) { cudaGraphExecDestroy(d.loop_exec); d.loop_exec = nullptr; }
        const long l0 = *launches;
        cudaGraph_t graph = nullptr;
        bool ok = cudaStreamBeginCapture(st, cudaStreamCaptureModeThreadLocal) == cudaSuccess;
        const int rc = ok ? run_loop() : 1;
        if (ok) ok = cudaStreamEndCapture(st, &graph) == cudaSuccess && graph != nullptr && rc == 0;
        if (ok) ok = cudaGraphInstantiate(&d.loop_exec, graph, 0) == cudaSuccess;
        if (graph != nullptr) cudaGraphDestroy(graph);
        if (!ok) {
            (void)cudaGetLastError();
            d.loop_exec = nullptr;
            d.graph_broken = true;
            *launches = l0;
            if (run_loop()) return 1;
        } else {
            d.loop_launches = *launches - l0;
            memcpy(d.loop_key, key, sizeof(key));
            CAPB_CHECK_CUDA(cudaGraphLaunch(d.loop_exec, st));
            if (debug) fprintf(stderr, "capb200: beam loop captured into a CUDA graph (%ld launches)\n", d.loop_launches);
        }
    } else {
        memcpy(d.seen_key, key, sizeof(key));
        if (run_loop()) return 1;
    }
    return 0;
}

template <class CoreFn>
int beam_decode_driver(DecodeBuffers& d, int V1, int T, int B, int beam, int keep, int penalty_kind, float penalty_alpha, long long* seq,
                       float* seq_logprobs, long long* done_seq, int* done_len, float* done_p, float* done_raw, CoreFn core, long* launches,
                       cudaStream_t st, unsigned long long graph_key = 0, const DecodeEdits& ed = DecodeEdits(), float temperature = 1.0f) {
    const int rows = B * beam;
    const bool edits = ed.any();
    const int k_in = beam + ed.kinds();
    CAPB_REQUIRE(!ed.trigrams, "block_trigrams applies to _sample only (AttModel.py:306)");
    CAPB_REQUIRE(k_in <= 16, "beam_size + number of active decode edits (decoding_constraint, remove_bad_endings, UNK suppression) must be <= 16");
    if (temperature == 0.f) temperature = 1.0f;
    CAPB_REQUIRE(temperature > 0.f, "temperature must be positive");
    if (grow_buffer(reinterpret_cast<void**>(&d.slab), &d.slab_bytes, (size_t)T * rows * V1 * sizeof(float), st)) return 1;
    d.slab_step_stride = (long)rows * V1;
    d.last_B = B;
    d.last_beam = beam;
    BeamState s = d.bs;
    s.B = B; s.beam = beam; s.T = T; s.V1 = V1;
    auto run_loop = [&]() -> int {
        CAPB_NVTX("capb200 beam loop (T steps: core, vocab stats, beam step)");
        CAPB_CHECK_CUDA(cudaMemsetAsync(s.sums, 0, sizeof(float) * B * beam, st));
        CAPB_CHECK_CUDA(cudaMemsetAsync(s.done_cnt, 0, sizeof(int) * B, st));
        CAPB_CHECK_CUDA(cudaMemsetAsync(d.tokens, 0, sizeof(int) * rows, st));
        for (int t = 0; t < T; ++t) {
            const int live = (t == 0) ? 1 : beam;
            const int nrows = B * live;
            float* logits = d.slab + (long)t * d.slab_step_stride;
            if (core(nrows, live, d.tokens, t == 0 ? d.neg1 : d.src_row, t, logits, (long)V1)) return 1;
            if (t > 0 && temperature != 1.0f) {
                if (scale_rows_launch(logits, V1, nrows, V1, 1.0f / temperature, st)) return 1;
                *launches += 1;
            }
            VocabStepArgs va;
            va.rows = nrows; va.V1 = V1; va.logits = logits; va.ld = V1;
            va.twice = (t > 0) ? 1 : 0;
            va.topk = edits ? k_in : beam; va.top_val = d.top_val; va.top_idx = d.top_idx;
            va.stats = d.slab_stats + (long)t * rows;
            if (vocab_step_launch(va, st)) return 1;
            const float* tv = d.top_val;
            const int* ti = d.top_idx;
            if (edits) {
                if (beam_edit_launch(nrows, k_in, beam, t, ed, d.tokens, d.top_val, d.top_idx, d.top_val_e, d.top_idx_e, st)) return 1;
                tv = d.top_val_e; ti = d.top_idx_e;
                *launches += 1;
            }
            if (beam_step_launch(s, t, live, tv, ti, penalty_kind, penalty_alpha, st)) return 1;
            *launches += 2;
        }
        return 0;
    };
    unsigned long long key[8] = {graph_key, (unsigned long long)B, (unsigned long long)beam, (unsigned long long)T, (unsigned long long)V1,
                                 (unsigned long long)penalty_kind, 0ull, (unsigned long long)reinterpret_cast<uintptr_t>(d.slab)};
    memcpy(&key[6], &penalty_alpha, sizeof(float));
    memcpy(reinterpret_cast<char*>(&key[6]) + 4, &temperature, sizeof(float));
    key[5] ^= ((unsigned long long)(ed.constraint & 1) << 8) ^ ((unsigned long long)(unsigned)(ed.unk_col + 1) << 16) ^ ((unsigned long long)ed.n_bad << 48);
    key[0] ^= (unsigned long long)reinterpret_cast<uintptr_t>(ed.bad) * 0x9E3779B97F4A7C15ull;
    d.last_edits = ed;
    d.last_stats = d.slab_stats;
    if (run_beam_loop(d, key, graph_key != 0, launches, st, run_loop)) return 1;
    CAPB_NVTX("capb200 beam finalize + log-prob rows");
    if (beam_finalize_launch(s, beam, d.rec_seq, d.rec_len, d.rec_p, d.rec_raw, d.rec_hist, st)) return 1;
    *launches += 1;
    if (keep == beam) {
        CAPB_CHECK_CUDA(cudaMemcpyAsync(seq, d.rec_seq, sizeof(long long) * B * beam * T, cudaMemcpyDeviceToDevice, st));
        if (seq_logprobs) {
            *launches += 1;
            if (gather_logprob_rows_launch(d.slab, d.slab_step_stride, V1, d.rec_hist, B * beam, T, V1, seq_logprobs, d.slab_stats, rows, st, d.rec_seq, &ed)) return 1;
        }
    } else {
        *launches += 1;
        if (beam_finalize_launch(s, 1, seq, d.tmp_len, d.tmp_p, d.tmp_raw, d.out_hist, st)) return 1;
        if (seq_logprobs) {
            *launches += 1;
            if (gather_logprob_rows_launch(d.slab, d.slab_step_stride, V1, d.out_hist, B, T, V1, seq_logprobs, d.slab_stats, rows, st, seq, &ed)) return 1;
        }
    }
    if (done_seq) CAPB_CHECK_CUDA(cudaMemcpyAsync(done_seq, d.rec_seq, sizeof(long long) * B * beam * T, cudaMemcpyDeviceToDevice, st));
    if (done_len) CAPB_CHECK_CUDA(cudaMemcpyAsync(done_len, d.rec_len, sizeof(int) * B * beam, cudaMemcpyDeviceToDevice, st));
    if (done_p) CAPB_CHECK_CUDA(cudaMemcpyAsync(done_p, d.rec_p, sizeof(float) * B * beam, cudaMemcpyDeviceToDevice, st));
    if (done_raw) CAPB_CHECK_CUDA(cudaMemcpyAsync(done_raw, d.rec_raw, sizeof(float) * B * beam, cudaMemcpyDeviceToDevice, st));
    return 0;
}

template <class CoreFn>
int diverse_beam_decode_driver(DecodeBuffers& d, int V1, int T, int B, int beam, int G, float lambda, int keep, int penalty_kind, float penalty_alpha,
                               long long* seq, float* seq_logprobs, long long* done_seq, int* done_len, float* done_p, float* done_raw, CoreFn core,
                               long* launches, cudaStream_t st, unsigned long long graph_key, const DecodeEdits& ed, float temperature) {
    CAPB_REQUIRE(G >= 2 && beam % G == 0, "diverse beam search needs group_size >= 2 dividing beam_size");
    CAPB_REQUIRE(lambda >= 0.f, "diversity_lambda must be >= 0");
    const int bdash = beam / G, rows = B * beam, steps = T + G - 1;
    CAPB_REQUIRE(keep == 1 || keep == bdash, "sample_n must be 1 or beam_size / group_size (AttModel.py:223)");
    const bool edits = ed.any();
    const int k_in = beam + ed.kinds();
    CAPB_REQUIRE(!ed.trigrams, "block_trigrams applies to _sample only (AttModel.py:306)");
    CAPB_REQUIRE(k_in <= 16, "beam_size + number of active decode edits (decoding_constraint, remove_bad_endings, UNK suppression) must be <= 16");
    if (temperature == 0.f) temperature = 1.0f;
    CAPB_REQUIRE(temperature > 0.f, "temperature must be positive");
    if (grow_buffer(reinterpret_cast<void**>(&d.slab), &d.slab_bytes, (size_t)steps * rows * V1 * sizeof(float), st)) return 1;
    if (grow_buffer(reinterpret_cast<void**>(&d.dbs_stats), &d.dbs_stats_bytes, (size_t)steps * rows * sizeof(float2), st)) return 1;
    if (grow_buffer(reinterpret_cast<void**>(&d.dbs_done_cnt), &d.dbs_done_bytes, (size_t)B * G * sizeof(int), st)) return 1;
    d.slab_step_stride = (long)rows * V1;
    d.last_B = B;
    d.last_beam = beam;
    d.last_edits = ed;
    d.last_stats = d.dbs_stats;
    BeamState s = d.bs;
    s.B = B * G; s.beam = bdash; s.T = T; s.V1 = V1;
    s.done_cnt = d.dbs_done_cnt;
    auto run_loop = [&]() -> int {
        CAPB_NVTX("capb200 diverse beam loop (T+G-1 steps: core, vocab stats, group steps)");
        CAPB_CHECK_CUDA(cudaMemsetAsync(s.sums, 0, sizeof(float) * rows, st));
        CAPB_CHECK_CUDA(cudaMemsetAsync(s.done_cnt, 0, sizeof(int) * B * G, st));
        CAPB_CHECK_CUDA(cudaMemsetAsync(d.tokens, 0, sizeof(int) * rows, st));
        CAPB_CHECK_CUDA(cudaMemsetAsync(d.src_row, 0xff, sizeof(int) * rows, st));
        for (int t = 0; t < steps; ++t) {
            float* logits = d.slab + (long)t * d.slab_step_stride;
            if (core(rows, beam, d.tokens, d.src_row, t, logits, (long)V1)) return 1;
            if (t > 0 && temperature != 1.0f) {
                if (scale_rows_launch(logits, V1, rows, V1, 1.0f / temperature, st, beam, bdash, t)) return 1;
                *launches += 1;
            }
            VocabStepArgs va;
            va.rows = rows; va.V1 = V1; va.logits = logits; va.ld = V1;
            va.twice = (t > 0) ? 1 : 0;
            va.first_beam = beam; va.first_group_rows = bdash; va.first_group = t;
            va.topk = edits ? k_in : beam; va.top_val = d.top_val; va.top_idx = d.top_idx;
            va.stats = d.dbs_stats + (long)t * rows;
            if (vocab_step_launch(va, st)) return 1;
            const float* tv = d.top_val;
            const int* ti = d.top_idx;
            if (edits) {
                if (beam_edit_launch(rows, k_in, beam, t, ed, d.tokens, d.top_val, d.top_idx, d.top_val_e, d.top_idx_e, st, beam, bdash, t)) return 1;
                tv = d.top_val_e; ti = d.top_idx_e;
                *launches += 1;
            }
            if (diverse_beam_step_launch(s, G, t, beam, tv, ti, lambda, rows, penalty_kind, penalty_alpha, st)) return 1;
            *launches += 2;
        }
        return 0;
// ... 251 lines not shown
```

### imagecaptioning.pytorch_b200/csrc/gemm_tc.cu

```cuda
#include <cstdlib>
#include <cstring>

#include "common.cuh"
#include "ptx.cuh"

namespace capb200 {

namespace {

constexpr int BM = 128;
constexpr int BK = 64;
constexpr int kConsumers = 2;
constexpr int kThreads = 128 * (1 + kConsumers);

struct TcParams {
    CUtensorMap a_hi[kMaxSeg];
    CUtensorMap a_lo[kMaxSeg];
    CUtensorMap w_hi[kMaxSeg];
    CUtensorMap w_lo[kMaxSeg];
    int kblocks[kMaxSeg];
    int nseg;
    int M, N;
    float* C;
    long ldc;
    __half* C_hi;
    __half* C_lo;
    long ldcs;
    const float* bias;
    const float* row_bias;
    long ld_row_bias;
    int rows_per_group;
    int relu;
    const float* residual;
    long ld_res;
    int tiles_m, tiles_n;
    int lstm, H;
    const float* c_prev;
    long ld_cprev;
    const int* src_row;
    float* c_out;
    long ld_cout;
    const float* gather_bias;
    long ld_gb;
    const int* gather_idx;
    float* h_f;
    __half* h_hi;
    __half* h_lo;
    long ld_h;
    unsigned long long* trace;
};

__device__ __forceinline__ unsigned long long gtimer() {
    unsigned long long t;
    asm volatile("mov.u64 %0, %%globaltimer;" : "=l"(t));
    return t;
}
#define CAPB_TRACE(slot) do { if (TRACE && p.trace != nullptr) p.trace[(long)blockIdx.x * 16 + (slot)] = gtimer(); } while (0)

template <int BN, int PASSES, int TM = BM>
struct TcCfg {
    static constexpr int kTileM = TM;
    static constexpr int kPasses = PASSES;
    static constexpr int kPlanes = (PASSES == 3) ? 2 : 1;
    static constexpr uint32_t kABytes = TM * BK * 2;
    static constexpr uint32_t kWBytes = BN * BK * 2;
    static constexpr uint32_t kStageBytes = kPlanes * (kABytes + kWBytes);
    static constexpr uint32_t kRingBudget = 227 * 1024 - 1024  - 256 ;
    static constexpr int kStages = kRingBudget / kStageBytes >= 8 ? 8 : kRingBudget / kStageBytes;
    static constexpr uint32_t kSmemBytes = kStages * kStageBytes + 1024  + 256 ;
    static_assert(BN == 64 || BN == 128 || BN == 160, "wgmma wrappers exist for N = 64, 128 and 160");
    static_assert(TM == BM || TM == 2 * BM, "one or two 128-row A boxes per plane");
    static_assert(kWBytes % 1024 == 0, "operand tiles must keep the 1024-byte swizzle-atom alignment");
    static_assert(kStages >= 2, "need at least a double buffer");
    static_assert(kSmemBytes <= 227 * 1024, "shared memory of one H100 block");
};

template <int BN>
__device__ __forceinline__ void wgmma_f16(float* acc, uint64_t da, uint64_t db, int scale_d) {
    if (BN == 160) ptx::wgmma_f16_n160(acc, da, db, scale_d);
    else if (BN == 128) ptx::wgmma_f16_n128(acc, da, db, scale_d);
    else ptx::wgmma_f16_n64(acc, da, db, scale_d);
}

enum EpiKind : int {
    kEpiStore = 0,
    kEpiPlanes = 1,
    kEpiLstm = 2,
};

template <int BN>
__device__ __forceinline__ void epi_adds(const TcParams& p, float* acc, int r0, int c0) {
    const int ncol = p.N - c0;
    const int lim[2] = {r0 < p.M ? ncol : 0, r0 + 8 < p.M ? ncol : 0};
    if (p.bias != nullptr) {
        const float* b = p.bias + c0;
#pragma unroll
        for (int j = 0; j < BN / 8; ++j) {
#pragma unroll
            for (int e = 0; e < 2; ++e) {
                if (8 * j + e < ncol) {
                    const float x = __ldg(b + 8 * j + e);
                    acc[4 * j + e] += x;
                    acc[4 * j + 2 + e] += x;
                }
            }
        }
    }
    const float* tab[3][2];
#pragma unroll
    for (int h = 0; h < 2; ++h) {
        const int row = lim[h] > 0 ? r0 + 8 * h : 0;
        tab[0][h] = p.row_bias != nullptr ? p.row_bias + (long)(row / p.rows_per_group) * p.ld_row_bias + c0 : nullptr;
        tab[1][h] = p.gather_bias != nullptr ? p.gather_bias + (long)(lim[h] > 0 ? p.gather_idx[row] : 0) * p.ld_gb + c0 : nullptr;
        tab[2][h] = p.residual != nullptr ? p.residual + (long)row * p.ld_res + c0 : nullptr;
    }
#pragma unroll 1
    for (int t = 0; t < 3; ++t) {
        const float* const t0 = t == 0 ? tab[0][0] : t == 1 ? tab[1][0] : tab[2][0];
        const float* const t1 = t == 0 ? tab[0][1] : t == 1 ? tab[1][1] : tab[2][1];
        if (t0 == nullptr) continue;
#pragma unroll
        for (int j = 0; j < BN / 8; ++j) {
#pragma unroll
            for (int e = 0; e < 4; ++e) {
                const int k = 8 * j + (e & 1);
                if (k < lim[e >> 1]) acc[4 * j + e] += (e >> 1 ? t1 : t0)[k];
            }
        }
    }
    if (p.relu) {
#pragma unroll
        for (int i = 0; i < BN / 2; ++i) acc[i] = fmaxf(acc[i], 0.0f);
    }
}

template <int BN, bool TRACE>
__device__ __forceinline__ void epi_lstm(const TcParams& p, float* acc, int r0, int c0, int lane, int slot) {
    constexpr int kRuns = BN / 32;
    const bool odd = lane & 1;
    const bool upper = lane & 2;
    const int row = r0 + (odd ? 8 : 0);
    const int u0 = ((c0 - 2 * (lane & 3)) >> 2) + (upper ? 4 : 0);
    const bool row_ok = row < p.M;
    const bool full = u0 + 8 * (kRuns - 1) + 4 <= p.H;
    int src = row;
    if (p.src_row != nullptr && row_ok) src = p.src_row[row];
    const float* cprev = (row_ok && src >= 0 && p.c_prev != nullptr) ? p.c_prev + (long)src * p.ld_cprev + u0 : nullptr;
    float cp[BN / 8];
    if (cprev != nullptr && full && (reinterpret_cast<uintptr_t>(cprev) & 15) == 0) {
#pragma unroll
        for (int k = 0; k < kRuns; ++k) {
            const float4 v = *reinterpret_cast<const float4*>(cprev + 8 * k);
            cp[4 * k] = v.x; cp[4 * k + 1] = v.y; cp[4 * k + 2] = v.z; cp[4 * k + 3] = v.w;
        }
    } else {
#pragma unroll
        for (int i = 0; i < BN / 8; ++i) {
            const int du = 8 * (i / 4) + i % 4;
            cp[i] = (cprev != nullptr && u0 + du < p.H) ? cprev[du] : 0.0f;
        }
    }
    if (TRACE && slot >= 0) {
        float s = 0.0f;
#pragma unroll
        for (int i = 0; i < BN / 8; ++i) s += cp[i];
        asm volatile("" ::"f"(s));
        CAPB_TRACE(slot);
    }
    __syncwarp();
#pragma unroll
// ... 46 lines not shown
#pragma unroll
            for (int k = 0; k < kRuns; ++k) {
                const float* c = cn + 4 * k;
                const float* h = hn + 4 * k;
                *reinterpret_cast<float4*>(c_out + 8 * k) = make_float4(c[0], c[1], c[2], c[3]);
                *reinterpret_cast<float4*>(h_f + 8 * k) = make_float4(h[0], h[1], h[2], h[3]);
                if (planes) {
                    __half hh[4], hl[4];
#pragma unroll
                    for (int o = 0; o < 4; ++o) split_f32(h[o], hh[o], hl[o]);
                    const __half2 hi01 = __halves2half2(hh[0], hh[1]), hi23 = __halves2half2(hh[2], hh[3]);
                    const __half2 lo01 = __halves2half2(hl[0], hl[1]), lo23 = __halves2half2(hl[2], hl[3]);
                    *reinterpret_cast<uint2*>(h_hi + 8 * k) = make_uint2(*reinterpret_cast<const uint32_t*>(&hi01), *reinterpret_cast<const uint32_t*>(&hi23));
                    *reinterpret_cast<uint2*>(h_lo + 8 * k) = make_uint2(*reinterpret_cast<const uint32_t*>(&lo01), *reinterpret_cast<const uint32_t*>(&lo23));
                }
            }
        } else {
#pragma unroll
            for (int i = 0; i < BN / 8; ++i) {
                const int du = 8 * (i / 4) + i % 4;
                if (u0 + du < p.H) {
                    c_out[du] = cn[i];
                    h_f[du] = hn[i];
                    if (planes) {
                        __half hh, hl;
                        split_f32(hn[i], hh, hl);
                        h_hi[du] = hh;
                        h_lo[du] = hl;
                    }
                }
            }
        }
    }
    if (TRACE && slot >= 0) CAPB_TRACE(slot + 2);
}

template <int BN, bool PLANES>
__device__ __forceinline__ void epi_store(const TcParams& p, const float* acc, int r0, int c0) {
    const int ncol = p.N - c0;
#pragma unroll
    for (int h = 0; h < 2; ++h) {
        const int row = r0 + 8 * h;
        if (row >= p.M) continue;
        if (p.C != nullptr) {
            float* const dst = p.C + (long)row * p.ldc + c0;
            if (ncol >= BN && (reinterpret_cast<uintptr_t>(dst) & 7) == 0) {
#pragma unroll
                for (int j = 0; j < BN / 8; ++j) *reinterpret_cast<float2*>(dst + 8 * j) = make_float2(acc[4 * j + 2 * h], acc[4 * j + 2 * h + 1]);
            } else {
#pragma unroll
                for (int j = 0; j < BN / 8; ++j) {
                    if (8 * j < ncol) dst[8 * j] = acc[4 * j + 2 * h];
                    if (8 * j + 1 < ncol) dst[8 * j + 1] = acc[4 * j + 2 * h + 1];
                }
            }
        }
        if (PLANES) {
            __half* const dh = p.C_hi + (long)row * p.ldcs + c0;
            __half* const dl = p.C_lo + (long)row * p.ldcs + c0;
            if (ncol >= BN && ((reinterpret_cast<uintptr_t>(dh) | reinterpret_cast<uintptr_t>(dl)) & 3) == 0) {
#pragma unroll
                for (int j = 0; j < BN / 8; ++j) {
                    __half h0, l0, h1, l1;
                    split_f32(acc[4 * j + 2 * h], h0, l0);
                    split_f32(acc[4 * j + 2 * h + 1], h1, l1);
                    *reinterpret_cast<__half2*>(dh + 8 * j) = __halves2half2(h0, h1);
                    *reinterpret_cast<__half2*>(dl + 8 * j) = __halves2half2(l0, l1);
                }
            } else {
#pragma unroll
                for (int j = 0; j < BN / 8; ++j) {
#pragma unroll
                    for (int e = 0; e < 2; ++e) {
                        __half hi, lo;
                        split_f32(acc[4 * j + 2 * h + e], hi, lo);
                        if (8 * j + e < ncol) { dh[8 * j + e] = hi; dl[8 * j + e] = lo; }
                    }
                }
            }
        }
    }
}

template <int BN, int EPI, bool TRACE>
__device__ __forceinline__ void epilogue_tile(const TcParams& p, float* acc, int m0, int n0, int tid, int slot) {
    const int warp = tid >> 5, lane = tid & 31;
    const int r0 = m0 + warp * 16 + (lane >> 2);
    const int c0 = n0 + 2 * (lane & 3);
    epi_adds<BN>(p, acc, r0, c0);
    if (EPI == kEpiLstm) epi_lstm<BN, TRACE>(p, acc, r0, c0, lane, slot);
    else epi_store<BN, EPI == kEpiPlanes>(p, acc, r0, c0);
}

template <int BN, int EPI, bool TRACE>
__device__ __forceinline__ void epilogue_rows128(const TcParams& p, float* acc0, const float* acc1, int m0, int n0, int tid, int slot) {
#pragma unroll 1
    for (int h = 0; h < 2; ++h) {
        epilogue_tile<BN, EPI, TRACE>(p, acc0, m0 + 64 * h, n0, tid, h == 0 ? slot : -1);
#pragma unroll
        for (int i = 0; i < BN / 2; ++i) acc0[i] = acc1[i];
    }
}

template <int PASSES>
__device__ __forceinline__ void init_ring(const TcParams& p, uint64_t* full_bar, uint64_t* empty_bar, int stages, int readers) {
    for (int s = 0; s < p.nseg; ++s) {
        ptx::prefetch_tmap(&p.a_hi[s]);
        ptx::prefetch_tmap(&p.w_hi[s]);
        if (PASSES == 3) {
            ptx::prefetch_tmap(&p.a_lo[s]);
            ptx::prefetch_tmap(&p.w_lo[s]);
        }
    }
    for (int i = 0; i < stages; ++i) {
        ptx::mbar_init(&full_bar[i], 1);
        ptx::mbar_init(&empty_bar[i], readers);
    }
}

template <typename Cfg>
__device__ __forceinline__ void fill_stage(const TcParams& p, uint8_t* st, uint64_t* bar, int s, int kb, int m0, int n0) {
    uint8_t* a_hi = st;
    uint8_t* a_lo = st + Cfg::kABytes;
    uint8_t* w_hi = st + Cfg::kABytes * Cfg::kPlanes;
    uint8_t* w_lo = w_hi + Cfg::kWBytes;
    ptx::mbar_arrive_expect_tx(bar, Cfg::kStageBytes);
#pragma unroll
    for (int r = 0; r < Cfg::kTileM; r += BM) ptx::tma_load_2d(a_hi + r * BK * 2, &p.a_hi[s], bar, kb * BK, m0 + r);
    ptx::tma_load_2d(w_hi, &p.w_hi[s], bar, kb * BK, n0);
    if (Cfg::kPasses == 3) {
#pragma unroll
        for (int r = 0; r < Cfg::kTileM; r += BM) ptx::tma_load_2d(a_lo + r * BK * 2, &p.a_lo[s], bar, kb * BK, m0 + r);
        ptx::tma_load_2d(w_lo, &p.w_lo[s], bar, kb * BK, n0);
    }
}

template <int BN, int PASSES>
__device__ __forceinline__ void mma_kblock(float* acc0, float* acc1, uint32_t a_hi, uint32_t a_lo, uint32_t w_hi, uint32_t w_lo) {
    constexpr uint32_t kHalf = 64 * 128;
#pragma unroll
    for (int i = 0; i < BN / 2; ++i) { ptx::reg_fence(acc0[i]); ptx::reg_fence(acc1[i]); }
    ptx::wgmma_fence();
#pragma unroll
    for (int k = 0; k < BK / 16; ++k) {
        const uint32_t koff = k * 32;
        const uint64_t dwh = ptx::make_smem_desc_sw128(w_hi + koff);
        if (PASSES == 3) {
            const uint64_t dwl = ptx::make_smem_desc_sw128(w_lo + koff);
            wgmma_f16<BN>(acc0, ptx::make_smem_desc_sw128(a_hi + koff), dwl, 1);
            wgmma_f16<BN>(acc1, ptx::make_smem_desc_sw128(a_hi + kHalf + koff), dwl, 1);
            wgmma_f16<BN>(acc0, ptx::make_smem_desc_sw128(a_lo + koff), dwh, 1);
            wgmma_f16<BN>(acc1, ptx::make_smem_desc_sw128(a_lo + kHalf + koff), dwh, 1);
            wgmma_f16<BN>(acc0, ptx::make_smem_desc_sw128(a_hi + koff), dwh, 1);
            wgmma_f16<BN>(acc1, ptx::make_smem_desc_sw128(a_hi + kHalf + koff), dwh, 1);
        } else {
            wgmma_f16<BN>(acc0, ptx::make_smem_desc_sw128(a_hi + koff), dwh, 1);
            wgmma_f16<BN>(acc1, ptx::make_smem_desc_sw128(a_hi + kHalf + koff), dwh, 1);
        }
    }
    ptx::wgmma_commit();
    ptx::wgmma_wait<0>();
#pragma unroll
    for (int i = 0; i < BN / 2; ++i) { ptx::reg_fence(acc0[i]); ptx::reg_fence(acc1[i]); }
}

template <int BN, int PASSES, int EPI, bool TRACE = false>
__global__ void __launch_bounds__(kThreads, 1) gemm_tc_kernel(const __grid_constant__ TcParams p) {
    using Cfg = TcCfg<BN, PASSES>;
    extern __shared__ uint8_t smem_raw[];
    uint8_t* smem = reinterpret_cast<uint8_t*>((reinterpret_cast<uintptr_t>(smem_raw) + 1023) & ~uintptr_t(1023));
    uint64_t* full_bar = reinterpret_cast<uint64_t*>(smem + Cfg::kStages * Cfg::kStageBytes);
    uint64_t* empty_bar = full_bar + Cfg::kStages;
    uint64_t* turn_bar = empty_bar + Cfg::kStages;

    const int wg = threadIdx.x >> 7;
    const int n_tiles = p.tiles_m * p.tiles_n;

    if (threadIdx.x == 0) {
        init_ring<PASSES>(p, full_bar, empty_bar, Cfg::kStages, 1);
        for (int c = 0; c < kConsumers; ++c) ptx::mbar_init(&turn_bar[c], 1);
        ptx::fence_mbar_init();
    }
    __syncthreads();
    if (threadIdx.x == 0) CAPB_TRACE(0);

    if (wg == 0) {
        ptx::setmaxnreg_dec<40>();
        if (threadIdx.x == 0) {
            int stage = 0;
            uint32_t phase = 0;
            for (int t = blockIdx.x; t < n_tiles; t += gridDim.x) {
                const int m0 = (t % p.tiles_m) * BM;
                const int n0 = (t / p.tiles_m) * BN;
                for (int s = 0; s < p.nseg; ++s) {
                    for (int kb = 0; kb < p.kblocks[s]; ++kb) {
                        ptx::mbar_wait(&empty_bar[stage], phase ^ 1);
                        fill_stage<Cfg>(p, smem + stage * Cfg::kStageBytes, &full_bar[stage], s, kb, m0, n0);
                        if (++stage == Cfg::kStages) { stage = 0; phase ^= 1; }
                    }
                }
            }
        }
    } else {
        ptx::setmaxnreg_inc<232>();
        const int cw = wg - 1;
        const int tid = threadIdx.x & 127;
        int kb_tile = 0;
        for (int s = 0; s < p.nseg; ++s) kb_tile += p.kblocks[s];
        int mine = 0;
        for (int it = cw, t = blockIdx.x + cw * gridDim.x; t < n_tiles; it += 2, t += 2 * gridDim.x, ++mine) {
            const int m0 = (t % p.tiles_m) * BM;
            const int n0 = (t / p.tiles_m) * BN;
            if (it > 0) ptx::mbar_wait(&turn_bar[cw], (cw == 1 ? mine : mine - 1) & 1);
            if (TRACE && it == 1 && tid == 0) CAPB_TRACE(4);
            const long g0 = (long)it * kb_tile;
            int stage = (int)(g0 % Cfg::kStages);
            uint32_t phase = (uint32_t)(g0 / Cfg::kStages) & 1;
            float acc0[BN / 2], acc1[BN / 2];
#pragma unroll
            for (int i = 0; i < BN / 2; ++i) { acc0[i] = 0.0f; acc1[i] = 0.0f; }
            for (int s = 0; s < p.nseg; ++s) {
                for (int kb = 0; kb < p.kblocks[s]; ++kb) {
                    ptx::mbar_wait(&full_bar[stage], phase);
                    if (TRACE && it == 0 && s == 0 && kb == 0 && tid == 0) CAPB_TRACE(1);
                    const uint32_t st = ptx::smem_u32(smem + stage * Cfg::kStageBytes);
                    const uint32_t w_hi = st + Cfg::kABytes * Cfg::kPlanes;
                    mma_kblock<BN, PASSES>(acc0, acc1, st, st + Cfg::kABytes, w_hi, w_hi + Cfg::kWBytes);
                    if (tid == 0) ptx::mbar_arrive(&empty_bar[stage]);
                    if (++stage == Cfg::kStages) { stage = 0; phase ^= 1; }
                }
            }
            if (tid == 0) ptx::mbar_arrive(&turn_bar[cw ^ 1]);
            if (TRACE && it < 2 && tid == 0) CAPB_TRACE(2 + it);
            epilogue_rows128<BN, EPI, TRACE>(p, acc0, acc1, m0, n0, tid, (TRACE && it < 2 && tid == 0) ? 9 + 3 * it : -1);
            if (TRACE && it < 2 && tid == 0) CAPB_TRACE(6 + it);
        }
    }
    __syncthreads();
    if (threadIdx.x == 0) CAPB_TRACE(8);
}

template <int BN, int PASSES, int EPI, bool TRACE = false>
__global__ void __launch_bounds__(kThreads, 1) gemm_tc256_kernel(const __grid_constant__ TcParams p) {
    using Cfg = TcCfg<BN, PASSES, 2 * BM>;
    extern __shared__ uint8_t smem_raw[];
    uint8_t* smem = reinterpret_cast<uint8_t*>((reinterpret_cast<uintptr_t>(smem_raw) + 1023) & ~uintptr_t(1023));
    uint64_t* full_bar = reinterpret_cast<uint64_t*>(smem + Cfg::kStages * Cfg::kStageBytes);
    uint64_t* empty_bar = full_bar + Cfg::kStages;

    const int wg = threadIdx.x >> 7;
    const int n_tiles = p.tiles_m * p.tiles_n;

    if (threadIdx.x == 0) {
        init_ring<PASSES>(p, full_bar, empty_bar, Cfg::kStages, kConsumers);
        ptx::fence_mbar_init();
    }
    __syncthreads();
    if (threadIdx.x == 0) CAPB_TRACE(0);

    if (wg == 0) {
        ptx::setmaxnreg_dec<40>();
        if (threadIdx.x == 0) {
            int stage = 0;
            uint32_t phase = 0;
            for (int t = blockIdx.x; t < n_tiles; t += gridDim.x) {
                const int m0 = (t % p.tiles_m) * Cfg::kTileM;
                const int n0 = (t / p.tiles_m) * BN;
                for (int s = 0; s < p.nseg; ++s) {
                    for (int kb = 0; kb < p.kblocks[s]; ++kb) {
                        ptx::mbar_wait(&empty_bar[stage], phase ^ 1);
                        fill_stage<Cfg>(p, smem + stage * Cfg::kStageBytes, &full_bar[stage], s, kb, m0, n0);
                        if (++stage == Cfg::kStages) { stage = 0; phase ^= 1; }
                    }
                }
                if (TRACE && t == (int)blockIdx.x) CAPB_TRACE(5);
            }
        }
    } else {
        ptx::setmaxnreg_inc<232>();
        const int cw = wg - 1;
        const int tid = threadIdx.x & 127;
        const uint32_t a_rows = cw * BM * BK * 2;
        int stage = 0;
        uint32_t phase = 0;
        for (int it = 0, t = blockIdx.x; t < n_tiles; ++it, t += gridDim.x) {
            const int m0 = (t % p.tiles_m) * Cfg::kTileM + BM * cw;
            const int n0 = (t / p.tiles_m) * BN;
            float acc0[BN / 2], acc1[BN / 2];
#pragma unroll
            for (int i = 0; i < BN / 2; ++i) { acc0[i] = 0.0f; acc1[i] = 0.0f; }
            for (int s = 0; s < p.nseg; ++s) {
                for (int kb = 0; kb < p.kblocks[s]; ++kb) {
                    ptx::mbar_wait(&full_bar[stage], phase);
                    if (TRACE && it == 0 && s == 0 && kb == 0 && cw == 0 && tid == 0) CAPB_TRACE(1);
                    const uint32_t st = ptx::smem_u32(smem + stage * Cfg::kStageBytes);
                    const uint32_t w_hi = st + Cfg::kABytes * Cfg::kPlanes;
                    mma_kblock<BN, PASSES>(acc0, acc1, st + a_rows, st + Cfg::kABytes + a_rows, w_hi, w_hi + Cfg::kWBytes);
                    if (tid == 0) ptx::mbar_arrive(&empty_bar[stage]);
                    if (++stage == Cfg::kStages) { stage = 0; phase ^= 1; }
                }
            }
            if (TRACE && it == 0 && tid == 0) CAPB_TRACE(2 + cw);
            epilogue_rows128<BN, EPI, TRACE>(p, acc0, acc1, m0, n0, tid, (TRACE && it == 0 && tid == 0) ? 9 + 3 * cw : -1);
            if (TRACE && it == 0 && tid == 0) CAPB_TRACE(6 + cw);
        }
    }
    __syncthreads();
    if (threadIdx.x == 0) CAPB_TRACE(8);
}

typedef CUresult (*EncodeTiledFn)(CUtensorMap*, CUtensorMapDataType, cuuint32_t, void*, const cuuint64_t*, const cuuint64_t*,
                                  const cuuint32_t*, const cuuint32_t*, CUtensorMapInterleave, CUtensorMapSwizzle,
                                  CUtensorMapL2promotion, CUtensorMapFloatOOBfill);

EncodeTiledFn get_encode_fn() {
    static EncodeTiledFn fn = nullptr;
    if (fn == nullptr) {
        void* sym = nullptr;
        cudaDriverEntryPointQueryResult qres;
        if (cudaGetDriverEntryPoint("cuTensorMapEncodeTiled", &sym, cudaEnableDefault, &qres) != cudaSuccess || sym == nullptr) {
            return nullptr;
        }
        fn = reinterpret_cast<EncodeTiledFn>(sym);
    }
    return fn;
}

bool encode_plane(CUtensorMap* map, const __half* base, long rows, long K, long pitch, int box_rows, std::string* err) {
    EncodeTiledFn fn = get_encode_fn();
    if (fn == nullptr) { *err = "cuTensorMapEncodeTiled entry point not available"; return false; }
    cuuint64_t gdim[2] = {static_cast<cuuint64_t>(K), static_cast<cuuint64_t>(rows)};
    cuuint64_t gstride[1] = {static_cast<cuuint64_t>(pitch) * 2};
    cuuint32_t box[2] = {static_cast<cuuint32_t>(BK), static_cast<cuuint32_t>(box_rows)};
    cuuint32_t estr[2] = {1, 1};
    CUresult r = fn(map, CU_TENSOR_MAP_DATA_TYPE_FLOAT16, 2, const_cast<__half*>(base), gdim, gstride, box, estr,
                    CU_TENSOR_MAP_INTERLEAVE_NONE, CU_TENSOR_MAP_SWIZZLE_128B, CU_TENSOR_MAP_L2_PROMOTION_L2_256B,
                    CU_TENSOR_MAP_FLOAT_OOB_FILL_NONE);
    if (r != CUDA_SUCCESS) { *err = "cuTensorMapEncodeTiled failed with CUresult " + std::to_string((int)r); return false; }
    return true;
}

template <int BN, int PASSES, int EPI, bool TRACE, int TM>
int launch_cfg(const TcParams& prm, cudaStream_t stream) {
    using Cfg = TcCfg<BN, PASSES, TM>;
    void (*kernel)(TcParams);
    if constexpr (TM == BM) kernel = gemm_tc_kernel<BN, PASSES, EPI, TRACE>;
    else kernel = gemm_tc256_kernel<BN, PASSES, EPI, TRACE>;
    static std::atomic<unsigned long long> attr_set{0};
    if (first_use_on_device(attr_set)) {
        CAPB_CHECK_CUDA(cudaFuncSetAttribute(kernel, cudaFuncAttributeMaxDynamicSharedMemorySize, Cfg::kSmemBytes));
    }
    TcParams prm2 = prm;
    prm2.tiles_n = cdiv(prm.N, BN);
    prm2.tiles_m = cdiv(prm.M, TM);
    const int n_tiles = prm2.tiles_n * prm2.tiles_m;
    const int sms = sm_count();
    kernel<<<n_tiles < sms ? n_tiles : sms, kThreads, Cfg::kSmemBytes, stream>>>(prm2);
    CAPB_CHECK_CUDA(cudaGetLastError());
    return 0;
}

template <int EPI, int TM>
int launch_width(int bn, int passes, const TcParams& prm, cudaStream_t stream) {
    if (prm.trace != nullptr) {
        if (bn == 160) return launch_cfg<160, 3, EPI, true, TM>(prm, stream);
        if constexpr (TM == BM) if (bn == 64) return launch_cfg<64, 3, EPI, true, TM>(prm, stream);
        return launch_cfg<128, 3, EPI, true, TM>(prm, stream);
    }
    if (bn == 160) return passes == 3 ? launch_cfg<160, 3, EPI, false, TM>(prm, stream) : launch_cfg<160, 1, EPI, false, TM>(prm, stream);
    if constexpr (TM == BM) {
        if (bn == 64) return passes == 3 ? launch_cfg<64, 3, EPI, false, TM>(prm, stream) : launch_cfg<64, 1, EPI, false, TM>(prm, stream);
    }
    return passes == 3 ? launch_cfg<128, 3, EPI, false, TM>(prm, stream) : launch_cfg<128, 1, EPI, false, TM>(prm, stream);
}

template <int EPI>
int launch_kind(int bm, int bn, int passes, const TcParams& prm, cudaStream_t stream) {
    return bm == 2 * BM ? launch_width<EPI, 2 * BM>(bn, passes, prm, stream) : launch_width<EPI, BM>(bn, passes, prm, stream);
}

}

struct GemmTcPlan {
    TcParams prm;
    int passes;
    int bn;
};

static void fill_epilogue(TcParams& t, const GemmEpilogue& e) {
    t.C = e.C; t.ldc = e.ldc;
    t.C_hi = e.C_hi; t.C_lo = e.C_lo; t.ldcs = e.ldcs;
    t.bias = e.bias; t.row_bias = e.row_bias; t.ld_row_bias = e.ld_row_bias;
    t.rows_per_group = e.rows_per_group < 1 ? 1 : e.rows_per_group;
    t.relu = e.relu;
    t.residual = e.residual; t.ld_res = e.ld_res;
    t.lstm = e.lstm; t.H = e.H;
    t.c_prev = e.c_prev; t.ld_cprev = e.ld_cprev; t.src_row = e.src_row;
    t.c_out = e.c_out; t.ld_cout = e.ld_cout;
    t.gather_bias = e.gather_bias; t.ld_gb = e.ld_gb; t.gather_idx = e.gather_idx;
    t.h_f = e.h_f; t.h_hi = e.h_hi; t.h_lo = e.h_lo; t.ld_h = e.ld_h;
    t.trace = e.trace;
}

bool gemm_tc_supported(const GemmProblem& p, std::string* why) {
    auto bad = [&](const char* m) { if (why) *why = m; return false; };
    if (p.nseg < 1 || p.nseg > kMaxSeg) return bad("1..3 K-segments");
    for (int s = 0; s < p.nseg; ++s) {
        const GemmSeg& g = p.seg[s];
        if (g.A_hi == nullptr || g.W_hi == nullptr) return bad("split planes missing");
        if ((g.lda_h & 7) || (g.ldw_h & 7)) return bad("plane pitch must be a multiple of 8 elements (16 bytes)");
        if ((reinterpret_cast<uintptr_t>(g.A_hi) & 15) || (reinterpret_cast<uintptr_t>(g.W_hi) & 15)) return bad("plane base must be 16-byte aligned");
        if (g.K < 1) return bad("empty K-segment");
    }
    return true;
}

int gemm_tc_tile_n(int M, int N) {
    const int sms = sm_count();
    const int tiles_m = cdiv(M, BM);
    if (tiles_m * cdiv(N, 128) < sms / 2 && N > 64) return 64;
    const long cost128 = (long)cdiv(tiles_m * cdiv(N, 128), sms) * 128;
    const long cost160 = (long)cdiv(tiles_m * cdiv(N, 160), sms) * 160;
    return cost160 < cost128 ? 160 : 128;
}

int gemm_tc_tile_m(int M, int N, int bn) {
    if (bn == 64) return BM;
    const char* force = getenv("CAPB200_GEMM_BM");
    if (force != nullptr && strcmp(force, "128") == 0) return BM;
    if (force != nullptr && strcmp(force, "256") == 0) return 2 * BM;
    const int sms = sm_count();
    const int tiles_n = cdiv(N, bn);
    return cdiv(M, 2 * BM) * tiles_n <= sms && cdiv(M, BM) * tiles_n > sms ? 2 * BM : BM;
}

GemmTcPlan* gemm_tc_plan_create(const GemmProblem& p, int passes) {
    std::string why;
    if (!gemm_tc_supported(p, &why)) { set_error("gemm_tc: unsupported problem: " + why); return nullptr; }
    if (passes != 1 && passes != 3) { set_error("gemm_tc: passes must be 1 or 3"); return nullptr; }
    GemmTcPlan* plan = new GemmTcPlan();
    memset(&plan->prm, 0, sizeof(TcParams));
    plan->passes = passes;
    plan->bn = gemm_tc_tile_n(p.M, p.N);
    TcParams& t = plan->prm;
    t.nseg = p.nseg;
    t.M = p.M;
    t.N = p.N;
    std::string err;
    for (int s = 0; s < p.nseg; ++s) {
        const GemmSeg& g = p.seg[s];
        t.kblocks[s] = cdiv(g.K, BK);
        bool ok = encode_plane(&t.a_hi[s], g.A_hi, p.M, g.K, g.lda_h, BM, &err) &&
                  encode_plane(&t.w_hi[s], g.W_hi, p.N, g.K, g.ldw_h, plan->bn, &err);
        if (ok && passes == 3) {
            if (g.A_lo == nullptr || g.W_lo == nullptr) { err = "lo planes missing for 3-pass mode"; ok = false; }
            ok = ok && encode_plane(&t.a_lo[s], g.A_lo, p.M, g.K, g.lda_h, BM, &err) &&
                 encode_plane(&t.w_lo[s], g.W_lo, p.N, g.K, g.ldw_h, plan->bn, &err);
        }
        if (!ok) { set_error("gemm_tc: " + err); delete plan; return nullptr; }
    }
    fill_epilogue(t, p.epi);
    return plan;
}

void gemm_tc_plan_destroy(GemmTcPlan* plan) { delete plan; }

int gemm_tc_plan_launch(GemmTcPlan* plan, const GemmEpilogue* epi_override, int M_override, cudaStream_t stream) {
    if (M_override > plan->prm.M) { set_error("gemm_tc: M override exceeds the planned row count"); return 1; }
    const int M = M_override > 0 ? M_override : plan->prm.M;
    TcParams prm = plan->prm;
    if (epi_override != nullptr) fill_epilogue(prm, *epi_override);
    prm.M = M;
    if (prm.lstm && (prm.N != 4 * prm.H || prm.c_out == nullptr || prm.h_f == nullptr)) {
        set_error("gemm_tc: fused LSTM epilogue needs N == 4H, c_out and h_f");
        return 1;
    }
    if (prm.M <= 0 || prm.N <= 0) return 0;
    const int kind = prm.lstm ? kEpiLstm : prm.C_hi != nullptr ? kEpiPlanes : kEpiStore;
    if (prm.trace != nullptr && plan->passes != 3) { set_error("gemm_tc: the traced kernel is the 3-pass one"); return 1; }
    const int bm = gemm_tc_tile_m(prm.M, prm.N, plan->bn);
    if (kind == kEpiLstm) return launch_kind<kEpiLstm>(bm, plan->bn, plan->passes, prm, stream);
    if (kind == kEpiPlanes) return launch_kind<kEpiPlanes>(bm, plan->bn, plan->passes, prm, stream);
    return launch_kind<kEpiStore>(bm, plan->bn, plan->passes, prm, stream);
}

}
```

### imagecaptioning.pytorch_b200/csrc/kernels.cuh

```cuda
#pragma once
#include "common.cuh"

namespace capb200 {

struct ActView {
    float* f = nullptr;
    __half* hi = nullptr;
    __half* lo = nullptr;
    long ld = 0;
};

struct StateCopy {
    const float* src = nullptr;
    long ld_src = 0;
    ActView dst;
};

int state_gather_embed_launch(int rows, const int* tokens, const int* src_row, const float* emb, long ld_emb, int E, int relu,
                              ActView xt, int H, int nstate, StateCopy sc0, StateCopy sc1, cudaStream_t stream);
int lstm_pointwise_launch(int rows, int H, const float* gates, long ld_g, const int* src_row, const float* c_prev, long ld_cp,
                          float* c_out, long ld_co, ActView h_out, const float* gather_bias, long ld_gb, const int* gather_idx,
                          cudaStream_t stream);
int relu_copy_launch(const float* x, long n, ActView out_flat, cudaStream_t stream);
int lstm_ln_launch(int rows, int H, const float* gates, long ld_g, const float* c_prev, long ld_cp, float* c_out, long ld_co, float* h_out, long ld_h,
                   const float* ln_a, const float* ln_b, float eps, float* ln_out, long ld_ln, cudaStream_t stream);
int maxout_pointwise_launch(int rows, int H, const float* sums, long ld_s, const int* src_row, const float* c_prev, long ld_cp,
                            float* c_out, long ld_co, ActView h_out, cudaStream_t stream);
int additive_attention_launch(int n_images, int rpi, int R, int A, int H, const float* att_h, long ld_ah, const float* p_att, long ld_pa,
                              const float* att, long ld_at, const float* mask, long ld_mask, const float* alpha_w, const float* alpha_b,
                              float* score_scratch , ActView out, cudaStream_t stream, float* alpha_out = nullptr );
int mask_rows_launch(ActView x, int n_images, int R, int cols, const float* mask, long ld_mask, cudaStream_t stream);
int ss_select_launch(int rows, int V1, const float* prev_logp, long ld, const long long* labels, long ld_labels, int col, unsigned long long seed, float prob,
                     int* tok_out, cudaStream_t stream);

struct DecodeEdits {
    int constraint = 0;
    int unk_col = -1;
    int n_bad = 0;
    const int* bad = nullptr;
    int trigrams = 0;
    int trigram_rows = 0;
    __host__ __device__ bool any() const { return constraint != 0 || unk_col >= 0 || n_bad > 0 || trigrams != 0; }
    __host__ __device__ int kinds() const { return (constraint ? 1 : 0) + (unk_col >= 0 ? 1 : 0) + (n_bad > 0 ? 1 : 0); }
};

struct VocabStepArgs {
    int rows = 0;
    int V1 = 0;
    float* logits = nullptr;
    long ld = 0;
    int twice = 0;
    float2* stats = nullptr;
    int topk = 0;
    float* top_val = nullptr;
    int* top_idx = nullptr;
    int select = 0;
    float top = 0.f;
    DecodeEdits edits;
    const int* prev_tokens = nullptr;
    float temperature = 1.0f;
    unsigned long long seed = 0;
    unsigned long long step = 0;
    const int* forced = nullptr;
    int* unfinished = nullptr;
    int first_step = 0;
    int* tokens_out = nullptr;
    long long* seq_out = nullptr;
    long ld_seq = 0;
    int t = 0;
    float* picked_lp = nullptr;
    long ld_picked = 1;
    int first_beam = 0, first_group_rows = 1, first_group = -1;
    __host__ __device__ int row_twice(int r) const {
        return twice && !(first_beam > 0 && (r % first_beam) / first_group_rows == first_group);
    }
};
int vocab_step_launch(const VocabStepArgs& a, cudaStream_t stream);
int beam_edit_launch(int rows, int k_in, int beam, int t, const DecodeEdits& ed, const int* prev_tokens, const float* val_in, const int* idx_in,
                     float* val_out, int* idx_out, cudaStream_t stream, int first_beam = 0, int first_group_rows = 1, int first_group = -1);
int scale_rows_launch(float* x, long ld, int rows, int cols, float factor, cudaStream_t stream, int skip_beam = 0, int skip_group_rows = 1,
                      int skip_group = -1);

struct BeamState {
    int B = 0, beam = 0, T = 0, V1 = 0;
    float* sums = nullptr;
    int* seq_a = nullptr;
    int* seq_b = nullptr;
    int* hist_a = nullptr;
    int* hist_b = nullptr;
    int* done_cnt = nullptr;
    int* done_seq = nullptr;
    int* done_hist = nullptr;
    int* done_len = nullptr;
    double* done_p = nullptr;
    float* done_raw = nullptr;
    int* tokens = nullptr;
    int* src_row = nullptr;
};
int beam_step_launch(const BeamState& s, int t, int live, const float* top_val, const int* top_idx, int penalty_kind, float penalty_alpha,
                     cudaStream_t stream);
int diverse_beam_step_launch(const BeamState& s, int G, int t, int k, const float* top_val, const int* top_idx, float lambda, int rows_total,
                             int penalty_kind, float penalty_alpha, cudaStream_t stream);
int beam_finalize_launch(const BeamState& s, int keep, long long* out_seq, int* out_len, float* out_p, float* out_raw, int* out_hist,
                         cudaStream_t stream);
int gather_logprob_rows_launch(const float* slab, long step_stride, long ld_slab, const int* hist, int nseq, int T, int V1, float* dst,
                               const float2* stats, long stats_stride, cudaStream_t stream, const long long* seqs = nullptr,
                               const DecodeEdits* ed = nullptr);

int layer_norm_launch(int rows, int D, const float* x, long ld_x, const float* a, const float* b, float eps, ActView out, cudaStream_t st);
int embed_pe_launch(int rows, int D, const int* tokens, const float* lut, const float* pe_row, float scale, ActView out, cudaStream_t st);
int enc_self_attention_launch(int B, int R, int heads, int dk, const float* q, const float* k, const float* v, long ld, const float* mask,
                              long ld_mask, ActView out, cudaStream_t st);
int dec_self_attention_launch(int rows, int heads, int dk, int t, const float* qkv, long ld_qkv, float* kcache, float* vcache, long step_stride,
                              long ld_c, const int* anc, long ld_anc, const long long* labels, long ld_lab, ActView out, cudaStream_t st);
int cross_attention_launch(int rows, int rpi, int heads, int dk, int R, const float* q, long ld_q, const float* kk, const float* vv, long ld_kv,
                           const float* mask, long ld_mask, ActView out, cudaStream_t st);

int glu_launch(int rows, int H, const float* t, long ld_t, const float* residual, long ld_res, ActView out, cudaStream_t st);
int masked_mean_launch(int B, int R, int H, const float* x, long ld_x, const float* mask, long ld_mask, ActView out, cudaStream_t st);

int gemm_generic_launch(int ta, int tb, int M, int N, int K, const float* A, long lda, const float* B, long ldb, float* C, long ldc, int accumulate,
                        const float* bias, cudaStream_t st);
int gemm_skinny_launch(int M, int N, int nseg, const float* const* A, const long* lda, const float* const* B, const long* ldb, const int* K, const int* tb,
                       float* C, long ldc, const float* bias, const float* row_bias, long ld_rb, int rpg, int accumulate, float* scratch,
                       size_t scratch_floats, int mode, cudaStream_t st);
int gemm_wgrad_launch(int M, int N, int K, const float* dY, long ld_dy, const float* X, long ld_x, float* G, long ld_g, int accumulate, int mode,
                      cudaStream_t st);
int colsum_launch(int rows, int cols, const float* x, long ld, float* out, int accumulate, cudaStream_t st);
struct Tf32Context;
Tf32Context* tf32_context_create();
void tf32_context_destroy(Tf32Context* c);
void tf32_context_new_step(Tf32Context* c);
long tf32_context_launches(const Tf32Context* c);
bool gemm_tf32_supported(int nseg, const float* const* X, const long* ldx, const float* const* W, const long* ldw, const int* K);
int gemm_tf32_launch(Tf32Context* ctx, int M, int N, int nseg, const float* const* X, const long* ldx, const float* const* W, const long* ldw, const int* K,
                     float* C, long ldc, const float* bias, const float* row_bias, long ld_rb, int rpg, int accumulate, cudaStream_t st);
const float* tf32_transposed(Tf32Context* ctx, const float* src, long ld_src, int rows, int cols, bool per_step, long* ld_dst, cudaStream_t st);
int dropout_apply_launch(float* x, int rows, int cols, long ld, unsigned long long seed, unsigned site, unsigned step, float p, cudaStream_t st);
int dropout_mask_launch(float* m, long n, unsigned long long seed, unsigned site, unsigned step, float p, cudaStream_t st);
int dropout_copy_launch(const float* x, long ld_x, float* y, long ld_y, int rows, int cols, unsigned long long seed, unsigned site, unsigned step, float p,
                        cudaStream_t st);
int embed_relu_dropout_launch(int rows, int E, const int* tokens, const float* emb, float* xt, unsigned long long seed, unsigned step, float p,
                              cudaStream_t st);
int scst_dlogits_launch(const float* logp, long ld_row, const long long* seq, const float* reward, const float* mask_sum, float upstream, int N, int T, int V1,
                        float* dl, cudaStream_t st, const float* row_coef = nullptr);
int scst_drop_worst_launch(const long long* seq, const float* row_loss, int N, int T, int keep, float upstream, float* row_msum, float* row_coef, float* loss,
                           cudaStream_t st);
int xe_loss_backward_launch(const float* logp, long ld_row, const long long* labels, long ld_l, const float* masks, long ld_m, int N, int steps, int Ls, int V1,
                            float smoothing, float upstream, float* mask_sum, float* item_loss, float* dl, float* loss, cudaStream_t st, int keep = 0,
                            float* row_loss = nullptr, float* row_msum = nullptr, float* row_coef = nullptr);
int logsoftmax_vjp_launch(const float* logp, const float* g, long ld_row, const long long* seq, int N, int T, int V1, float* dl, cudaStream_t st);
int lstm_cell_backward_launch(int rows, int H, const float* gates, const float* c_prev, const float* c_new, const float* dh, const float* dh_extra,
                              long ld_extra, unsigned drop_site, unsigned drop_step, unsigned long long seed, float p, float* dc_carry, float* dgates,
                              cudaStream_t st);
int maxout_cell_backward_launch(int rows, int H, const float* sums, const float* c_prev, const float* c_new, const float* dh, const float* dh_extra,
                                long ld_extra, unsigned drop_site, unsigned drop_step, unsigned long long seed, float p, float* dc_carry, float* dsums,
                                cudaStream_t st);
int attention_backward_launch(int n_images, int rpi, int R, int A, int H, const float* d_out, const float* alpha, const float* att_h, const float* p_att,
                              const float* att, const float* w, float* d_att_h, float* d_att, float* d_p_att, float* d_w, float* d_b, float* d_alpha_scratch,
                              cudaStream_t st);
// ... 81 lines not shown
```

### imagecaptioning.pytorch_b200/csrc/vocab.cu

```cuda
#include <cooperative_groups.h>
#include "common.cuh"
#include "kernels.cuh"

namespace cg = cooperative_groups;

namespace capb200 {

static __device__ unsigned long long g_vocab_seed_salt = 0ull;
int dropout_salt_set_vocab(unsigned long long salt, cudaStream_t st) {
    return cudaMemcpyToSymbolAsync(g_vocab_seed_salt, &salt, sizeof(salt), 0, cudaMemcpyHostToDevice, st) == cudaSuccess ? 0 : 1;
}

namespace {

constexpr int VT = 256;

template <int NT = VT>
__device__ __forceinline__ float block_max(float v, float* scratch) {
#pragma unroll
    for (int o = 16; o > 0; o >>= 1) v = fmaxf(v, __shfl_xor_sync(0xffffffffu, v, o));
    __syncthreads();
    if ((threadIdx.x & 31) == 0) scratch[threadIdx.x >> 5] = v;
    __syncthreads();
    float r = scratch[0];
// ... 434 lines not shown
    out_v = sval[0];
    out_i = sidx[0];
#pragma unroll
    for (int w = 1; w < VT2 / 32; ++w) {
        const float ov = sval[w];
        const int oi = sidx[w];
        if (ov > out_v || (ov == out_v && oi < out_i)) { out_v = ov; out_i = oi; }
    }
}

__global__ void __launch_bounds__(VT2) vocab_stats_online128_kernel(const VocabStepArgs a) {
    __shared__ float s_red[VT2 / 32];
    __shared__ int s_idx[VT2 / 32];
    const int r = blockIdx.x;
    const int n4 = a.V1 >> 2;
    const float4* g4 = reinterpret_cast<const float4*>(a.logits + (long)r * a.ld);
    constexpr float kL2E = 1.4426950408889634f;
    float t0v = -INFINITY, t1v = -INFINITY;
    int t0i = 0x7fffffff, t1i = 0x7fffffff;
    float m = -INFINITY, mL = -INFINITY, part = 0.f;
    auto consume = [&](const float4 x, int v) {
        const float m4 = fmaxf(fmaxf(x.x, x.y), fmaxf(x.z, x.w));
        if (m4 > m) {
            online_raise(part, m, mL, m4);
        }
        float e0, e1, e2, e3;
        asm("ex2.approx.ftz.f32 %0, %1;" : "=f"(e0) : "f"(fmaf(x.x, kL2E, -mL)));
        asm("ex2.approx.ftz.f32 %0, %1;" : "=f"(e1) : "f"(fmaf(x.y, kL2E, -mL)));
        asm("ex2.approx.ftz.f32 %0, %1;" : "=f"(e2) : "f"(fmaf(x.z, kL2E, -mL)));
        asm("ex2.approx.ftz.f32 %0, %1;" : "=f"(e3) : "f"(fmaf(x.w, kL2E, -mL)));
        part += (e0 + e1) + (e2 + e3);
        if (m4 > t1v) {
            const float xs[4] = {x.x, x.y, x.z, x.w};
#pragma unroll
            for (int u = 0; u < 4; ++u) {
                if (xs[u] > t1v) {
                    if (xs[u] > t0v) { t1v = t0v; t1i = t0i; t0v = xs[u]; t0i = 4 * v + u; }
                    else { t1v = xs[u]; t1i = 4 * v + u; }
                }
            }
        }
    };
    int v = threadIdx.x;
    for (; v + 3 * VT2 < n4; v += 4 * VT2) {
        const float4 x0 = g4[v], x1 = g4[v + VT2], x2 = g4[v + 2 * VT2], x3 = g4[v + 3 * VT2];
        consume(x0, v); consume(x1, v + VT2); consume(x2, v + 2 * VT2); consume(x3, v + 3 * VT2);
    }
    for (; v < n4; v += VT2) consume(g4[v], v);
    const float mx = block_max4(m, s_red);
    float sum = online_finish(part, m, mL, mx);
    sum = block_sum4(sum, s_red);
    const float lsum = logf(sum);
    const float m2 = (mx - mx) - lsum, l2 = lsum;
    if (threadIdx.x == 0) a.stats[r] = make_float2(mx, lsum);
    int popped = 0;
    for (int k = 0; k < a.topk; ++k) {
        float ov;
        int oi;
        block_argmax4(t0v, t0i, s_red, s_idx, ov, oi);
        if (t0i == oi && oi != 0x7fffffff) {
            const float lastv = t0v;
            const int lasti = t0i;
            t0v = t1v; t0i = t1i;
            t1v = -INFINITY; t1i = 0x7fffffff;
            if (++popped >= 2 && t0i == 0x7fffffff) {
                auto consider = [&](float x, int w) {
                    const bool after = (x < lastv) || (x == lastv && w > lasti);
                    if (after && (x > t0v || (x == t0v && w < t0i))) { t0v = x; t0i = w; }
                };
                for (int w = threadIdx.x; w < n4; w += VT2) {
                    const float4 x = g4[w];
                    consider(x.x, 4 * w); consider(x.y, 4 * w + 1); consider(x.z, 4 * w + 2); consider(x.w, 4 * w + 3);
                }
            }
        }
        if (threadIdx.x == 0) {
            const float lp = (ov - mx) - lsum;
            a.top_val[(long)r * a.topk + k] = a.row_twice(r) ? (lp - m2) - l2 : lp;
            a.top_idx[(long)r * a.topk + k] = oi;
        }
    }
}

__global__ void __launch_bounds__(VT) ss_select_kernel(int V1, const float* __restrict__ prev_logp, long ld, const long long* __restrict__ labels,
                                                      long ld_labels, int col, unsigned long long seed, float prob, int* __restrict__ tok_out) {
    __shared__ float s_red[VT / 32];
    __shared__ int s_idx[VT / 32];
    const int r = blockIdx.x;
    seed ^= g_vocab_seed_salt;
    const uint32_t k0 = (uint32_t)seed ^ 0x6a09e667u, k1 = (uint32_t)(seed >> 32) ^ 0xbb67ae85u;
    const uint32_t ubits = philox_first(0xffffffffu, (uint32_t)r, (uint32_t)col, 6u, k0, k1);
    const float u_row = ((float)(ubits >> 9) + 0.5f) * (1.0f / 8388608.0f);
    if (!(u_row < prob)) {
        if (threadIdx.x == 0) tok_out[r] = (int)labels[(long)r * ld_labels + col];
        return;
    }
    const float* g = prev_logp + (long)r * ld;
    float bv = -INFINITY;
    int bi = 0x7fffffff;
    for (int v = threadIdx.x; v < V1; v += VT) {
        const uint32_t bits = philox_first((uint32_t)v, (uint32_t)r, (uint32_t)col, 6u, k0, k1);
        const float u = ((float)(bits >> 9) + 0.5f) * (1.0f / 8388608.0f);
        const float x = g[v] - logf(-logf(u));
        if (x > bv) { bv = x; bi = v; }
    }
    float ov;
    int tok;
    block_argmax(bv, bi, s_red, s_idx, ov, tok);
    if (threadIdx.x == 0) tok_out[r] = tok;
}

__global__ void mask_rows_kernel(ActView x, int R, int cols, const float* __restrict__ mask, long ld_mask) {
    const int row = blockIdx.x;
    const int img = row / R, r = row % R;
    if (mask[(long)img * ld_mask + r] != 0.f) return;
    for (int c = threadIdx.x; c < cols; c += blockDim.x) {
        x.f[(long)row * x.ld + c] = 0.f;
        if (x.hi) { x.hi[(long)row * x.ld + c] = __float2half(0.f); x.lo[(long)row * x.ld + c] = __float2half(0.f); }
    }
}

template <int KMAX>
int vocab_step_cluster_launch_k(const VocabStepArgs& a, cudaStream_t stream) {
    const int C = cdiv(a.V1, kRowSmem);
    const int S = cdiv(a.V1, C);
    static std::atomic<unsigned long long> configured{0};
    if (first_use_on_device(configured)) {
        CAPB_CHECK_CUDA(cudaFuncSetAttribute(vocab_step_cluster_kernel<KMAX, VTC>, cudaFuncAttributeMaxDynamicSharedMemorySize,
                                             (int)(sizeof(float) * kRowSmem)));
    }
    cudaLaunchConfig_t cfg = {};
    cfg.gridDim = dim3((unsigned)(a.rows * C));
    cfg.blockDim = dim3(VTC);
    cfg.dynamicSmemBytes = sizeof(float) * (size_t)S;
    cfg.stream = stream;
    cudaLaunchAttribute attr[1];
    attr[0].id = cudaLaunchAttributeClusterDimension;
    attr[0].val.clusterDim.x = (unsigned)C;
    attr[0].val.clusterDim.y = 1;
    attr[0].val.clusterDim.z = 1;
    cfg.attrs = attr;
    cfg.numAttrs = 1;
    CAPB_CHECK_CUDA(cudaLaunchKernelEx(&cfg, vocab_step_cluster_kernel<KMAX, VTC>, a, S));
    return 0;
}

int vocab_step_cluster_launch(const VocabStepArgs& a, cudaStream_t stream) {
    if (a.topk <= 2) return vocab_step_cluster_launch_k<2>(a, stream);
    if (a.topk <= 8) return vocab_step_cluster_launch_k<8>(a, stream);
    return vocab_step_cluster_launch_k<16>(a, stream);
}

}

int vocab_step_launch(const VocabStepArgs& a, cudaStream_t stream) {
    if (a.rows <= 0) return 0;
    CAPB_REQUIRE(a.topk <= 16, "beam size up to 16");
    if (a.stats != nullptr) {
        CAPB_REQUIRE(a.select == 0 && a.topk > 0, "stats mode is the beam-search epilogue");
        const bool vec = ((a.V1 & 3) == 0) && ((a.ld & 3) == 0) && ((reinterpret_cast<uintptr_t>(a.logits) & 15) == 0);
        if (vec) vocab_stats_online128_kernel<<<a.rows, VT2, 0, stream>>>(a);
        else vocab_stats_kernel<<<a.rows, VT, 0, stream>>>(a);
        CAPB_CHECK_CUDA(cudaGetLastError());
        return 0;
    }
    CAPB_REQUIRE(a.V1 <= kMaxRow, "the vocabulary step supports up to 409600 entries per row (V + 1 <= 409600, a cluster of 8 CTAs "
                                  "caching 51200 entries each)");
    if (a.V1 > kRowSmem) return vocab_step_cluster_launch(a, stream);
    const size_t smem = sizeof(float) * (size_t)a.V1;
    static std::atomic<unsigned long long> configured{0};
    if (first_use_on_device(configured)) {
        CAPB_CHECK_CUDA(cudaFuncSetAttribute(vocab_step_kernel<2>, cudaFuncAttributeMaxDynamicSharedMemorySize, (int)(200 * 1024)));
        CAPB_CHECK_CUDA(cudaFuncSetAttribute(vocab_step_kernel<8>, cudaFuncAttributeMaxDynamicSharedMemorySize, (int)(200 * 1024)));
        CAPB_CHECK_CUDA(cudaFuncSetAttribute(vocab_step_kernel<16>, cudaFuncAttributeMaxDynamicSharedMemorySize, (int)(200 * 1024)));
    }
    if (a.topk <= 2 && a.select != 0 && a.rows <= 2 * sm_count()) {
        static std::atomic<unsigned long long> configured2{0};
        if (first_use_on_device(configured2)) {
            CAPB_CHECK_CUDA(cudaFuncSetAttribute(vocab_step_kernel<2, 1024>, cudaFuncAttributeMaxDynamicSharedMemorySize, (int)(200 * 1024)));
        }
        vocab_step_kernel<2, 1024><<<a.rows, 1024, smem, stream>>>(a);
    }
    else if (a.topk <= 2) vocab_step_kernel<2><<<a.rows, VT, smem, stream>>>(a);
    else if (a.topk <= 8) vocab_step_kernel<8><<<a.rows, VT, smem, stream>>>(a);
    else vocab_step_kernel<16><<<a.rows, VT, smem, stream>>>(a);
    CAPB_CHECK_CUDA(cudaGetLastError());
    return 0;
}

int ss_select_launch(int rows, int V1, const float* prev_logp, long ld, const long long* labels, long ld_labels, int col, unsigned long long seed, float prob,
                     int* tok_out, cudaStream_t stream) {
    if (rows <= 0) return 0;
    ss_select_kernel<<<rows, VT, 0, stream>>>(V1, prev_logp, ld, labels, ld_labels, col, seed, prob, tok_out);
    CAPB_CHECK_CUDA(cudaGetLastError());
    return 0;
}

int mask_rows_launch(ActView x, int n_images, int R, int cols, const float* mask, long ld_mask, cudaStream_t stream) {
    if (n_images <= 0 || mask == nullptr) return 0;
    mask_rows_kernel<<<n_images * R, 128, 0, stream>>>(x, R, cols, mask, ld_mask);
    CAPB_CHECK_CUDA(cudaGetLastError());
    return 0;
}

}
```

### include/capb200.h

```cpp
#ifndef CAPB200_H_
#define CAPB200_H_

#ifdef __cplusplus
extern "C" {
#endif

#define CAPB200_ABI_VERSION 1

#define CAPB200_MODE_SIMT_FP32 0
#define CAPB200_MODE_TC_F16X3 1
#define CAPB200_MODE_TC_F16X1 2
#define CAPB200_MODE_SKINNY_TF32X3 3
#define CAPB200_MODE_SKINNY_FP32 4
#define CAPB200_MODE_TF32X3_TC 5
#define CAPB200_MODE_TF32X3_TC_DGRAD 6
#define CAPB200_MODE_TF32X3_TC_WGRAD 7

#define CAPB200_FAMILY_UPDOWN 0
#define CAPB200_FAMILY_NEWFC 1
#define CAPB200_FAMILY_ATT2IN2 2

typedef struct capb200_engine capb200_engine;
typedef struct capb200_cider_table capb200_cider_table;

// ... 390 lines not shown
typedef struct {
    int sample_n;
    float temperature;
    unsigned long long seed;
    float upstream;
    int baseline;
    float drop_prob_lm, dropout;
    const long long* forced_tokens;
    const float* att_masks;
    int keep_rows;
    float* row_loss;
    const capb200_sampler_opts* sampler;
    const capb200_reward_weights* reward_weights;
} capb200_tfm_scst_opts;
int capb200_tfm_xe_step(capb200_tfm_engine* e, const float* att, int B, int R, const capb200_tfm_xe_opts* opts, const long long* labels, const float* masks,
                        int label_cols, const capb200_tfm_grads* grads, float* logprobs, float* loss, void* stream);
int capb200_tfm_scst_step(capb200_tfm_engine* e, const float* att, int B, int R, const capb200_tfm_scst_opts* opts, const capb200_cider_table* table,
                          const int* refs, const int* ref_offsets, int L, const capb200_tfm_grads* grads, long long* sample_seq, long long* greedy_seq,
                          float* sample_logprobs, float* reward, float* loss, void* stream);
int capb200_tfm_set_grad_events(capb200_tfm_engine* e, void* const* events, int n);

typedef struct {
    int forward_only;
    const float* dlogprobs;
    int greedy;
} capb200_vjp_opts;
int capb200_updown_xe_vjp(capb200_engine* e, const float* fc, const float* att, int B, int R, const capb200_xe_opts* opts, const capb200_vjp_opts* vjp,
                          const long long* labels, int label_cols, const capb200_updown_grads* grads, float* logprobs, void* stream);
int capb200_updown_scst_vjp(capb200_engine* e, const float* fc, const float* att, int B, int R, const capb200_scst_opts* opts, const capb200_vjp_opts* vjp,
                            const capb200_updown_grads* grads, long long* sample_seq, float* sample_logprobs, void* stream);
int capb200_att2in2_xe_vjp(capb200_engine* e, const float* fc, const float* att, int B, int R, const capb200_xe_opts* opts, const capb200_vjp_opts* vjp,
                           const long long* labels, int label_cols, const capb200_att2in2_grads* grads, float* logprobs, void* stream);
int capb200_att2in2_scst_vjp(capb200_engine* e, const float* fc, const float* att, int B, int R, const capb200_scst_opts* opts, const capb200_vjp_opts* vjp,
                             const capb200_att2in2_grads* grads, long long* sample_seq, float* sample_logprobs, void* stream);
int capb200_newfc_xe_vjp(capb200_engine* e, const float* fc, const float* att, int B, int R, const capb200_xe_opts* opts, const capb200_vjp_opts* vjp,
                         const long long* labels, int label_cols, const capb200_newfc_grads* grads, float* logprobs, void* stream);
int capb200_newfc_scst_vjp(capb200_engine* e, const float* fc, const float* att, int B, int R, const capb200_scst_opts* opts, const capb200_vjp_opts* vjp,
                           const capb200_newfc_grads* grads, long long* sample_seq, float* sample_logprobs, void* stream);
int capb200_aoa_xe_vjp(capb200_aoa_engine* e, const float* att, int B, int R, const capb200_aoa_xe_opts* opts, const capb200_vjp_opts* vjp,
                       const long long* labels, int label_cols, const capb200_aoa_grads* grads, float* logprobs, void* stream);
int capb200_aoa_scst_vjp(capb200_aoa_engine* e, const float* att, int B, int R, const capb200_aoa_scst_opts* opts, const capb200_vjp_opts* vjp,
                         const capb200_aoa_grads* grads, long long* sample_seq, float* sample_logprobs, void* stream);
int capb200_tfm_xe_vjp(capb200_tfm_engine* e, const float* att, int B, int R, const capb200_tfm_xe_opts* opts, const capb200_vjp_opts* vjp,
                       const long long* labels, int label_cols, const capb200_tfm_grads* grads, float* logprobs, void* stream);
int capb200_tfm_scst_vjp(capb200_tfm_engine* e, const float* att, int B, int R, const capb200_tfm_scst_opts* opts, const capb200_vjp_opts* vjp,
                         const capb200_tfm_grads* grads, long long* sample_seq, float* sample_logprobs, void* stream);

int capb200_adam_chunk_elems(void);
int capb200_adam_step(const unsigned long long* table, const long long* numel, const int* chunks, int n_chunks, double lr, double beta1, double beta2,
                      double eps, double weight_decay, long step, double clip_value, int write_clamped, void* stream);


typedef struct {
    const float* bias;
    const float* row_bias;
    long ld_row_bias;
    int rows_per_group;
    const float* residual;
    long ld_res;
    int relu;
    float* C;
    long ldc;
    unsigned short* C_hi;
    unsigned short* C_lo;
    long ldcs;
    int lstm;
    int H;
    const float* c_prev;
    long ld_cprev;
    const int* src_row;
    float* c_out;
    long ld_cout;
    const float* gather_bias;
    long ld_gb;
    const int* gather_idx;
    float* h_f;
    unsigned short* h_hi;
    unsigned short* h_lo;
    long ld_h;
} capb200_gemm_epilogue;
int capb200_decode_gemm(const float* x, const float* w, int M, int N, int K, int mode, const capb200_gemm_epilogue* epi, unsigned long long* trace_host,
                        int n_slots, void* stream);

#ifdef __cplusplus
}
#endif
#endif
```

Before: 23910.

## Fuse vocab softmax stats and top-k partials into logit GEMM epilogue

The logit GEMM epilogue now computes a per-tile row max, sum of exponentials and per-thread-quad best candidates, and writes them to a small partials buffer. A new lightweight merge kernel combines these into the log-sum-exp stats and the beam top-k, re-reading only the candidate columns from the logits. This replaces the full vocab_step pass over each logits row during beam search when temperature is 1 and no edits apply. It adds epilogue work and register pressure to the GEMM, and relies on exp2.approx for the partial sums.

```diff
diff --git a/imagecaptioning.pytorch_b200/_lib.py b/imagecaptioning.pytorch_b200/_lib.py
--- a/imagecaptioning.pytorch_b200/_lib.py
+++ b/imagecaptioning.pytorch_b200/_lib.py
@@ -289,6 +289,8 @@
     'capb200_reward_criterion_forward': (c_int, [c_void_p, c_void_p, c_void_p, c_int, c_int, c_int, c_void_p, c_void_p, c_void_p, c_void_p]),
     'capb200_reward_criterion_backward': (c_int, [c_void_p, c_void_p, c_int, c_int, c_int, c_void_p, c_float, c_void_p, c_void_p]),
     'capb200_decode_gemm': (c_int, [c_void_p, c_void_p, c_int, c_int, c_int, c_int, POINTER(GemmEpilogue), c_void_p, c_int, c_void_p]),
+    'capb200_logit_partials_topk': (c_int, [c_void_p, c_void_p, c_void_p, c_int, c_int, c_int, c_int, c_int, c_int, c_void_p, c_long,
+                                            c_void_p, c_void_p, c_void_p, c_void_p]),
     'capb200_updown_xe_vjp': (c_int, [c_void_p, c_void_p, c_void_p, c_int, c_int, POINTER(XeOpts), POINTER(VjpOpts), c_void_p, c_int,
                                       POINTER(UpdownGrads), c_void_p, c_void_p]),
     'capb200_updown_scst_vjp': (c_int, [c_void_p, c_void_p, c_void_p, c_int, c_int, POINTER(ScstOpts), POINTER(VjpOpts), POINTER(UpdownGrads),
diff --git a/imagecaptioning.pytorch_b200/csrc/aoa_engine.cu b/imagecaptioning.pytorch_b200/csrc/aoa_engine.cu
--- a/imagecaptioning.pytorch_b200/csrc/aoa_engine.cu
+++ b/imagecaptioning.pytorch_b200/csrc/aoa_engine.cu
@@ -117,6 +117,7 @@
     e->ld_c = round_up(H, 8);
     for (int i = 0; i < 2; ++i) e->c0[i] = a.take<float>((long)rows * e->ld_c);
     e->d.carve(a, B, rows, beam, T);
+    if (tc) e->d.carve_partials(a, rows, e->V1, gemm_tc_tile_n(rows, e->V1));
 }
 
 int ensure_workspace(capb200_aoa_engine* e, int B, int rows, int R, int beam, cudaStream_t st) {
@@ -280,6 +281,7 @@
     g.seg[0] = seg_of(e->ctx_out.v, w.logit_w, H, e->p_logit, H);
     g.epi.bias = w.logit_b;
     g.epi.C = logits; g.epi.ldc = ld_logits;
+    e->d.request_partials(g.epi);
     (void)B;
     return gemm(e, A_LOGIT, g, e->capRows, st);
 }
diff --git a/imagecaptioning.pytorch_b200/csrc/common.cuh b/imagecaptioning.pytorch_b200/csrc/common.cuh
--- a/imagecaptioning.pytorch_b200/csrc/common.cuh
+++ b/imagecaptioning.pytorch_b200/csrc/common.cuh
@@ -69,6 +69,7 @@
     long ldw_h = 0;
     int K = 0;
 };
+constexpr int kPartialWords = 10;
 struct GemmEpilogue {
     const float* bias = nullptr;
     const float* row_bias = nullptr;
@@ -96,6 +97,8 @@
     __half* h_hi = nullptr;
     __half* h_lo = nullptr;
     long ld_h = 0;
+    float* partials = nullptr;
+    int part_tiles = 0;
     unsigned long long* trace = nullptr;
 };
 
diff --git a/imagecaptioning.pytorch_b200/csrc/engine.cu b/imagecaptioning.pytorch_b200/csrc/engine.cu
--- a/imagecaptioning.pytorch_b200/csrc/engine.cu
+++ b/imagecaptioning.pytorch_b200/csrc/engine.cu
@@ -210,6 +210,7 @@
     e->img_of_row = a.take<int>(rows);
     e->att_score = a.take<float>((long)rows * (R > 0 ? R : 1));
     e->d.carve(a, B, rows, beam, T);
+    if (tc) e->d.carve_partials(a, rows, e->V1, gemm_tc_tile_n(rows, e->V1));
 }
 
 int ensure_workspace(capb200_engine* e, int B, int rows, int R, int beam, cudaStream_t st) {
@@ -400,6 +401,7 @@
             g.seg[0] = seg_of(e->h1_out.v, w.logit_w, H, e->p_logit, H);
             g.epi.bias = w.logit_b;
             g.epi.C = logits; g.epi.ldc = ld_logits;
+            e->d.request_partials(g.epi);
             if (run_gemm(e, G_LOGIT, g, e->capRows, st)) return 1;
         }
         return 0;
@@ -446,6 +448,7 @@
         g.seg[0] = seg_of(e->h0_out.v, w.logit_w, H, e->p_logit, H);
         g.epi.bias = w.logit_b;
         g.epi.C = logits; g.epi.ldc = ld_logits;
+        e->d.request_partials(g.epi);
         return run_gemm(e, G_LOGIT, g, e->capRows, st);
     }
     const bool fresh = (src_row == e->d.neg1);
@@ -476,6 +479,7 @@
     g.seg[0] = seg_of(e->h0_out.v, w.logit_w, H, e->p_logit, H);
     g.epi.bias = w.logit_b;
     g.epi.C = logits; g.epi.ldc = ld_logits;
+    e->d.request_partials(g.epi);
     return run_gemm(e, G_LOGIT, g, e->capRows, st);
 }
 
@@ -966,6 +970,43 @@
     if (plan) gemm_tc_plan_destroy(plan);
     cudaFree(scratch);
     if (trace) cudaFree(trace);
+    return rc;
+}
+
+int capb200_logit_partials_topk(const float* x, const float* w, const float* bias, int M, int N, int K, int mode, int twice, int k, float* C,
+                                long ldc, float* stats, float* top_val, int* top_idx, void* stream) {
+    cudaStream_t st = static_cast<cudaStream_t>(stream);
+    CAPB_REQUIRE(x && w && C && stats && top_val && top_idx && M > 0 && N > 0 && K > 0 && ldc >= N, "bad argument");
+    CAPB_REQUIRE(mode == CAPB200_MODE_TC_F16X3 || mode == CAPB200_MODE_TC_F16X1, "the decode GEMM runs in the tc_f16x3 / tc_f16x1 modes");
+    CAPB_REQUIRE(k >= 1 && k <= 16, "1 <= k <= 16");
+    const int bn = gemm_tc_tile_n(M, N), tiles = cdiv(N, bn);
+    GemmProblem g;
+    g.M = M; g.N = N; g.nseg = 1;
+    g.seg[0].K = K;
+    g.epi.bias = bias;
+    g.epi.C = C; g.epi.ldc = ldc;
+    const long ldh = round_up(K, 64);
+    __half* scratch = nullptr;
+    float* part = nullptr;
+    CAPB_CHECK_CUDA(cudaMalloc(&scratch, (size_t)(M + N) * ldh * 2 * sizeof(__half)));
+    if (cudaMalloc(&part, sizeof(float) * (size_t)M * tiles * kPartialWords) != cudaSuccess) {
+        cudaFree(scratch);
+        CAPB_CHECK_CUDA(cudaGetLastError());
+    }
+    g.epi.partials = part; g.epi.part_tiles = tiles;
+    __half* xh = scratch; __half* xl = xh + (size_t)M * ldh;
+    __half* wh = xl + (size_t)M * ldh; __half* wl = wh + (size_t)N * ldh;
+    int rc = split_planes_launch(x, K, M, K, xh, xl, ldh, st) | split_planes_launch(w, K, N, K, wh, wl, ldh, st);
+    g.seg[0].A_hi = xh; g.seg[0].A_lo = xl; g.seg[0].lda_h = ldh;
+    g.seg[0].W_hi = wh; g.seg[0].W_lo = wl; g.seg[0].ldw_h = ldh;
+    GemmTcPlan* plan = rc ? nullptr : gemm_tc_plan_create(g, mode == CAPB200_MODE_TC_F16X3 ? 3 : 1);
+    if (plan == nullptr) rc = 1;
+    if (!rc) rc = gemm_tc_plan_launch(plan, nullptr, 0, st);
+    if (!rc) rc = vocab_partials_merge_launch(M, part, tiles, bn, N, C, ldc, k, twice ? 1 : 0, reinterpret_cast<float2*>(stats), top_val, top_idx, st);
+    if (cudaStreamSynchronize(st) != cudaSuccess) { set_error(std::string("logit_partials_topk: ") + cudaGetErrorString(cudaGetLastError())); rc = 1; }
+    if (plan) gemm_tc_plan_destroy(plan);
+    cudaFree(scratch);
+    cudaFree(part);
     return rc;
 }
 
diff --git a/imagecaptioning.pytorch_b200/csrc/engine_common.cuh b/imagecaptioning.pytorch_b200/csrc/engine_common.cuh
--- a/imagecaptioning.pytorch_b200/csrc/engine_common.cuh
+++ b/imagecaptioning.pytorch_b200/csrc/engine_common.cuh
@@ -95,6 +95,9 @@
     float* top_val_e = nullptr;
     int* top_idx_e = nullptr;
     float2* slab_stats = nullptr;
+    float* partials = nullptr;
+    int part_tiles = 0, part_bn = 0;
+    bool part_req = false;
     BeamState bs;
     long long* rec_seq = nullptr;
     int *rec_len = nullptr, *rec_hist = nullptr, *out_hist = nullptr, *tmp_len = nullptr;
@@ -158,6 +161,17 @@
         tmp_p = a.take<float>((long)B * beam);
         tmp_raw = a.take<float>((long)B * beam);
     }
+
+    void carve_partials(Arena& a, int rows, int V1, int bn) {
+        part_bn = bn;
+        part_tiles = cdiv(V1, bn);
+        partials = a.take<float>((long)rows * part_tiles * kPartialWords);
+    }
+
+    void request_partials(GemmEpilogue& e) const {
+        if (!part_req) return;
+        e.partials = partials; e.part_tiles = part_tiles;
+    }
 };
 
 __global__ void capb_fill_int_kernel(int* p, int n, int v);
@@ -248,6 +262,7 @@
     d.last_beam = beam;
     BeamState s = d.bs;
     s.B = B; s.beam = beam; s.T = T; s.V1 = V1;
+    const bool fused = d.partials != nullptr && !edits && temperature == 1.0f;
     auto run_loop = [&]() -> int {
         CAPB_NVTX("capb200 beam loop (T steps: core, vocab stats, beam step)");
         CAPB_CHECK_CUDA(cudaMemsetAsync(s.sums, 0, sizeof(float) * B * beam, st));
@@ -257,7 +272,10 @@
             const int live = (t == 0) ? 1 : beam;
             const int nrows = B * live;
             float* logits = d.slab + (long)t * d.slab_step_stride;
-            if (core(nrows, live, d.tokens, t == 0 ? d.neg1 : d.src_row, t, logits, (long)V1)) return 1;
+            d.part_req = fused;
+            const int rc = core(nrows, live, d.tokens, t == 0 ? d.neg1 : d.src_row, t, logits, (long)V1);
+            d.part_req = false;
+            if (rc) return 1;
             if (t > 0 && temperature != 1.0f) {
                 if (scale_rows_launch(logits, V1, nrows, V1, 1.0f / temperature, st)) return 1;
                 *launches += 1;
@@ -267,7 +285,12 @@
             va.twice = (t > 0) ? 1 : 0;
             va.topk = edits ? k_in : beam; va.top_val = d.top_val; va.top_idx = d.top_idx;
             va.stats = d.slab_stats + (long)t * rows;
-            if (vocab_step_launch(va, st)) return 1;
+            if (fused) {
+                if (vocab_partials_merge_launch(nrows, d.partials, d.part_tiles, d.part_bn, V1, logits, V1, beam, va.twice, va.stats, d.top_val, d.top_idx,
+                                                st)) return 1;
+            } else if (vocab_step_launch(va, st)) {
+                return 1;
+            }
             const float* tv = d.top_val;
             const int* ti = d.top_idx;
             if (edits) {
@@ -286,6 +309,7 @@
     memcpy(reinterpret_cast<char*>(&key[6]) + 4, &temperature, sizeof(float));
     key[5] ^= ((unsigned long long)(ed.constraint & 1) << 8) ^ ((unsigned long long)(unsigned)(ed.unk_col + 1) << 16) ^ ((unsigned long long)ed.n_bad << 48);
     key[0] ^= (unsigned long long)reinterpret_cast<uintptr_t>(ed.bad) * 0x9E3779B97F4A7C15ull;
+    key[3] ^= (unsigned long long)fused << 32;
     d.last_edits = ed;
     d.last_stats = d.slab_stats;
     if (run_beam_loop(d, key, graph_key != 0, launches, st, run_loop)) return 1;
diff --git a/imagecaptioning.pytorch_b200/csrc/gemm_tc.cu b/imagecaptioning.pytorch_b200/csrc/gemm_tc.cu
--- a/imagecaptioning.pytorch_b200/csrc/gemm_tc.cu
+++ b/imagecaptioning.pytorch_b200/csrc/gemm_tc.cu
@@ -48,6 +48,8 @@
     __half* h_lo;
     long ld_h;
     unsigned long long* trace;
+    float* partials;
+    int part_tiles;
 };
 
 __device__ __forceinline__ unsigned long long gtimer() {
@@ -86,6 +88,7 @@
     kEpiStore = 0,
     kEpiPlanes = 1,
     kEpiLstm = 2,
+    kEpiVocab = 3,
 };
 
 template <int BN>
@@ -298,6 +301,61 @@
     }
 }
 
+template <int BN>
+__device__ __forceinline__ void epi_partials(const TcParams& p, float* acc, int r0, int c0, int n0) {
+    constexpr float kL2E = 1.4426950408889634f;
+    const int ncol = p.N - c0;
+    if (ncol < BN) {
+#pragma unroll
+        for (int j = 0; j < BN / 8; ++j) {
+#pragma unroll
+            for (int e = 0; e < 4; ++e) {
+                if (8 * j + (e & 1) >= ncol) acc[4 * j + e] = -INFINITY;
+            }
+        }
+    }
+    float bv[2] = {-INFINITY, -INFINITY};
+    int bo[2] = {0x7fffffff, 0x7fffffff};
+#pragma unroll
+    for (int j = 0; j < BN / 8; ++j) {
+#pragma unroll
+        for (int e = 0; e < 4; ++e) {
+            const float x = acc[4 * j + e];
+            if (x > bv[e >> 1]) { bv[e >> 1] = x; bo[e >> 1] = 8 * j + (e & 1); }
+        }
+    }
+    float m[2];
+#pragma unroll
+    for (int h = 0; h < 2; ++h) {
+        m[h] = fmaxf(bv[h], __shfl_xor_sync(0xffffffffu, bv[h], 1));
+        m[h] = fmaxf(m[h], __shfl_xor_sync(0xffffffffu, m[h], 2));
+    }
+    const float mL[2] = {m[0] * kL2E, m[1] * kL2E};
+    float s[2] = {0.f, 0.f};
+#pragma unroll
+    for (int j = 0; j < BN / 8; ++j) {
+#pragma unroll
+        for (int e = 0; e < 4; ++e) {
+            float x;
+            asm("ex2.approx.ftz.f32 %0, %1;" : "=f"(x) : "f"(fmaf(acc[4 * j + e], kL2E, -mL[e >> 1])));
+            s[e >> 1] += x;
+        }
+    }
+    const int q = (c0 - n0) >> 1;
+#pragma unroll
+    for (int h = 0; h < 2; ++h) {
+        s[h] += __shfl_xor_sync(0xffffffffu, s[h], 1);
+        s[h] += __shfl_xor_sync(0xffffffffu, s[h], 2);
+        const int row = r0 + 8 * h;
+        if (row < p.M) {
+            float* const dst = p.partials + ((long)row * p.part_tiles + n0 / BN) * kPartialWords;
+            if (q == 0) { dst[0] = m[h]; dst[1] = s[h]; }
+            dst[2 + q] = bv[h];
+            dst[6 + q] = __int_as_float(bo[h] == 0x7fffffff ? 0x7fffffff : c0 + bo[h]);
+        }
+    }
+}
+
 template <int BN, int EPI, bool TRACE>
 __device__ __forceinline__ void epilogue_tile(const TcParams& p, float* acc, int m0, int n0, int tid, int slot) {
     const int warp = tid >> 5, lane = tid & 31;
@@ -306,6 +364,7 @@
     epi_adds<BN>(p, acc, r0, c0);
     if (EPI == kEpiLstm) epi_lstm<BN, TRACE>(p, acc, r0, c0, lane, slot);
     else epi_store<BN, EPI == kEpiPlanes>(p, acc, r0, c0);
+    if (EPI == kEpiVocab) epi_partials<BN>(p, acc, r0, c0, n0);
 }
 
 template <int BN, int EPI, bool TRACE>
@@ -380,8 +439,8 @@
     for (int i = 0; i < BN / 2; ++i) { ptx::reg_fence(acc0[i]); ptx::reg_fence(acc1[i]); }
 }
 
-template <int BN, int PASSES, int EPI, bool TRACE = false>
-__global__ void __launch_bounds__(kThreads, 1) gemm_tc_kernel(const __grid_constant__ TcParams p) {
+template <int BN, int PASSES, int EPI, bool TRACE>
+__device__ __forceinline__ void pingpong_gemm(const TcParams& p) {
     using Cfg = TcCfg<BN, PASSES>;
     extern __shared__ uint8_t smem_raw[];
     uint8_t* smem = reinterpret_cast<uint8_t*>((reinterpret_cast<uintptr_t>(smem_raw) + 1023) & ~uintptr_t(1023));
@@ -457,6 +516,16 @@
 }
 
 template <int BN, int PASSES, int EPI, bool TRACE = false>
+__global__ void __launch_bounds__(kThreads, 1) gemm_tc_kernel(const __grid_constant__ TcParams p) {
+    pingpong_gemm<BN, PASSES, EPI, TRACE>(p);
+}
+
+template <int BN, int PASSES>
+__global__ void __launch_bounds__(kThreads, 1) gemm_tc_vocab_kernel(const __grid_constant__ TcParams p) {
+    pingpong_gemm<BN, PASSES, kEpiVocab, false>(p);
+}
+
+template <int BN, int PASSES, int EPI, bool TRACE = false>
 __global__ void __launch_bounds__(kThreads, 1) gemm_tc256_kernel(const __grid_constant__ TcParams p) {
     using Cfg = TcCfg<BN, PASSES, 2 * BM>;
     extern __shared__ uint8_t smem_raw[];
@@ -560,7 +629,8 @@
 int launch_cfg(const TcParams& prm, cudaStream_t stream) {
     using Cfg = TcCfg<BN, PASSES, TM>;
     void (*kernel)(TcParams);
-    if constexpr (TM == BM) kernel = gemm_tc_kernel<BN, PASSES, EPI, TRACE>;
+    if constexpr (EPI == kEpiVocab) kernel = gemm_tc_vocab_kernel<BN, PASSES>;
+    else if constexpr (TM == BM) kernel = gemm_tc_kernel<BN, PASSES, EPI, TRACE>;
     else kernel = gemm_tc256_kernel<BN, PASSES, EPI, TRACE>;
     static std::atomic<unsigned long long> attr_set{0};
     if (first_use_on_device(attr_set)) {
@@ -588,6 +658,12 @@
         if (bn == 64) return passes == 3 ? launch_cfg<64, 3, EPI, false, TM>(prm, stream) : launch_cfg<64, 1, EPI, false, TM>(prm, stream);
     }
     return passes == 3 ? launch_cfg<128, 3, EPI, false, TM>(prm, stream) : launch_cfg<128, 1, EPI, false, TM>(prm, stream);
+}
+
+int launch_vocab(int bn, int passes, const TcParams& prm, cudaStream_t stream) {
+    if (bn == 160) return passes == 3 ? launch_cfg<160, 3, kEpiVocab, false, BM>(prm, stream) : launch_cfg<160, 1, kEpiVocab, false, BM>(prm, stream);
+    if (bn == 64) return passes == 3 ? launch_cfg<64, 3, kEpiVocab, false, BM>(prm, stream) : launch_cfg<64, 1, kEpiVocab, false, BM>(prm, stream);
+    return passes == 3 ? launch_cfg<128, 3, kEpiVocab, false, BM>(prm, stream) : launch_cfg<128, 1, kEpiVocab, false, BM>(prm, stream);
 }
 
 template <int EPI>
@@ -615,6 +691,7 @@
     t.c_out = e.c_out; t.ld_cout = e.ld_cout;
     t.gather_bias = e.gather_bias; t.ld_gb = e.ld_gb; t.gather_idx = e.gather_idx;
     t.h_f = e.h_f; t.h_hi = e.h_hi; t.h_lo = e.h_lo; t.ld_h = e.ld_h;
+    t.partials = e.partials; t.part_tiles = e.part_tiles;
     t.trace = e.trace;
 }
 
@@ -694,6 +771,13 @@
     if (prm.M <= 0 || prm.N <= 0) return 0;
     const int kind = prm.lstm ? kEpiLstm : prm.C_hi != nullptr ? kEpiPlanes : kEpiStore;
     if (prm.trace != nullptr && plan->passes != 3) { set_error("gemm_tc: the traced kernel is the 3-pass one"); return 1; }
+    if (prm.partials != nullptr) {
+        if (prm.lstm || prm.C == nullptr || prm.C_hi != nullptr || prm.trace != nullptr || prm.part_tiles != cdiv(prm.N, plan->bn)) {
+            set_error("gemm_tc: row-statistics partials need fp32 C alone and part_tiles == the plan's column tiles");
+            return 1;
+        }
+        return launch_vocab(plan->bn, plan->passes, prm, stream);
+    }
     const int bm = gemm_tc_tile_m(prm.M, prm.N, plan->bn);
     if (kind == kEpiLstm) return launch_kind<kEpiLstm>(bm, plan->bn, plan->passes, prm, stream);
     if (kind == kEpiPlanes) return launch_kind<kEpiPlanes>(bm, plan->bn, plan->passes, prm, stream);
diff --git a/imagecaptioning.pytorch_b200/csrc/kernels.cuh b/imagecaptioning.pytorch_b200/csrc/kernels.cuh
--- a/imagecaptioning.pytorch_b200/csrc/kernels.cuh
+++ b/imagecaptioning.pytorch_b200/csrc/kernels.cuh
@@ -76,6 +76,8 @@
     }
 };
 int vocab_step_launch(const VocabStepArgs& a, cudaStream_t stream);
+int vocab_partials_merge_launch(int rows, const float* partials, int tiles, int bn, int V1, const float* logits, long ld, int k, int twice,
+                                float2* stats, float* top_val, int* top_idx, cudaStream_t stream);
 int beam_edit_launch(int rows, int k_in, int beam, int t, const DecodeEdits& ed, const int* prev_tokens, const float* val_in, const int* idx_in,
                      float* val_out, int* idx_out, cudaStream_t stream, int first_beam = 0, int first_group_rows = 1, int first_group = -1);
 int scale_rows_launch(float* x, long ld, int rows, int cols, float factor, cudaStream_t stream, int skip_beam = 0, int skip_group_rows = 1,
diff --git a/imagecaptioning.pytorch_b200/csrc/vocab.cu b/imagecaptioning.pytorch_b200/csrc/vocab.cu
--- a/imagecaptioning.pytorch_b200/csrc/vocab.cu
+++ b/imagecaptioning.pytorch_b200/csrc/vocab.cu
@@ -540,6 +540,116 @@
     }
 }
 
+constexpr int kMergeWarps = 4;
+constexpr int kMergeSeg = 40;
+__device__ __forceinline__ void warp_best(float& bv, int& bi) {
+#pragma unroll
+    for (int o = 16; o > 0; o >>= 1) {
+        const float v = __shfl_xor_sync(0xffffffffu, bv, o);
+        const int i = __shfl_xor_sync(0xffffffffu, bi, o);
+        if (v > bv || (v == bv && i < bi)) { bv = v; bi = i; }
+    }
+}
+__device__ __forceinline__ void offer(float v, int i, float lv, int li, float& bv, int& bi) {
+    const bool after = v < lv || (v == lv && i > li);
+    if (after && (v > bv || (v == bv && i < bi))) { bv = v; bi = i; }
+}
+
+__global__ void __launch_bounds__(32 * kMergeWarps) vocab_partials_merge_kernel(const float* __restrict__ part, int rows, int tiles, int bn,
+                                                                              int V1, const float* __restrict__ logits, long ld, int k,
+                                                                              int twice, float2* __restrict__ stats, float* __restrict__ top_val,
+                                                                              int* __restrict__ top_idx) {
+    __shared__ float s_val[kMergeWarps][16 * kMergeSeg];
+    __shared__ int s_col[kMergeWarps][16 * kMergeSeg];
+    constexpr float kL2E = 1.4426950408889634f;
+    const int warp = threadIdx.x >> 5, lane = threadIdx.x & 31;
+    const int r = blockIdx.x * kMergeWarps + warp;
+    if (r >= rows) return;
+    const float* pr = part + (long)r * tiles * kPartialWords;
+    const float* row = logits + (long)r * ld;
+    float mx = -INFINITY;
+    for (int t = lane; t < tiles; t += 32) mx = fmaxf(mx, pr[(long)t * kPartialWords]);
+#pragma unroll
+    for (int o = 16; o > 0; o >>= 1) mx = fmaxf(mx, __shfl_xor_sync(0xffffffffu, mx, o));
+    float sum = 0.f;
+    for (int t = lane; t < tiles; t += 32) {
+        const float mt = pr[(long)t * kPartialWords];
+        float sc;
+        asm("ex2.approx.ftz.f32 %0, %1;" : "=f"(sc) : "f"(fmaf(-mx, kL2E, mt * kL2E)));
+        sum += (mt == -INFINITY) ? 0.f : pr[(long)t * kPartialWords + 1] * sc;
+    }
+#pragma unroll
+    for (int o = 16; o > 0; o >>= 1) sum += __shfl_xor_sync(0xffffffffu, sum, o);
+    const float lsum = logf(sum);
+    const float m2 = (mx - mx) - lsum, l2 = lsum;
+    if (lane == 0) stats[r] = make_float2(mx, lsum);
+
+    auto seg_next = [&](float lv, int li, float& bv, int& bi) {
+        bv = -INFINITY; bi = 0x7fffffff;
+        for (int t = lane; t < tiles; t += 32) {
+            const float* pt = pr + (long)t * kPartialWords;
+#pragma unroll
+            for (int g = 0; g < 4; ++g) {
+                const int i = __float_as_int(pt[6 + g]);
+                if (i != 0x7fffffff) offer(pt[2 + g], i, lv, li, bv, bi);
+            }
+        }
+    };
+    const int per_seg = bn / 4;
+    float hv;
+    int hi;
+    seg_next(INFINITY, -1, hv, hi);
+    int npick = 0;
+    for (int q = 0; q < k; ++q) {
+        float bv = hv;
+        int bi = hi;
+        warp_best(bv, bi);
+        if (bi == 0x7fffffff) break;
+        if (lane == 0) s_col[warp][q] = bi;
+        if (hi == bi) seg_next(bv, bi, hv, hi);
+        ++npick;
+    }
+    __syncwarp();
+    const int nslot = npick * per_seg;
+    constexpr int kSlots = 16 * kMergeSeg / 32;
+    float val[kSlots];
+    int col[kSlots];
+#pragma unroll
+    for (int w = 0; w < kSlots; ++w) {
+        const int u = lane + 32 * w, p = u / per_seg, e = u - p * per_seg;
+        const int c = u < nslot ? s_col[warp][p] : 0;
+        const int n0 = c / bn * bn;
+        col[w] = n0 + ((c - n0) & 6) + 8 * (e >> 1) + (e & 1);
+        val[w] = (u < nslot && col[w] < V1) ? row[col[w]] : -INFINITY;
+    }
+    __syncwarp();
+#pragma unroll
+    for (int w = 0; w < kSlots; ++w) {
+        const int u = lane + 32 * w;
+        if (u < nslot) { s_val[warp][u] = val[w]; s_col[warp][u] = col[w]; }
+    }
+    __syncwarp();
+    auto slot_next = [&](float lv, int li, float& bv, int& bi) {
+        bv = -INFINITY; bi = 0x7fffffff;
+        for (int u = lane; u < nslot; u += 32) {
+            const float v = s_val[warp][u];
+            if (v > -INFINITY) offer(v, s_col[warp][u], lv, li, bv, bi);
+        }
+    };
+    slot_next(INFINITY, -1, hv, hi);
+    for (int q = 0; q < k; ++q) {
+        float bv = hv;
+        int bi = hi;
+        warp_best(bv, bi);
+        if (lane == 0) {
+            const float lp = (bv - mx) - lsum;
+            top_val[(long)r * k + q] = twice ? (lp - m2) - l2 : lp;
+            top_idx[(long)r * k + q] = bi;
+        }
+        if (hi == bi && bi != 0x7fffffff) slot_next(bv, bi, hv, hi);
+    }
+}
+
 __global__ void __launch_bounds__(VT) ss_select_kernel(int V1, const float* __restrict__ prev_logp, long ld, const long long* __restrict__ labels,
                                                       long ld_labels, int col, unsigned long long seed, float prob, int* __restrict__ tok_out) {
     __shared__ float s_red[VT / 32];
@@ -646,6 +756,16 @@
     return 0;
 }
 
+int vocab_partials_merge_launch(int rows, const float* partials, int tiles, int bn, int V1, const float* logits, long ld, int k, int twice,
+                                float2* stats, float* top_val, int* top_idx, cudaStream_t stream) {
+    if (rows <= 0) return 0;
+    CAPB_REQUIRE(k >= 1 && k <= 16 && bn % 8 == 0 && bn / 4 <= kMergeSeg && tiles == cdiv(V1, bn), "1 <= k <= 16, bn <= 160 and tiles == cdiv(V1, bn)");
+    vocab_partials_merge_kernel<<<cdiv(rows, kMergeWarps), 32 * kMergeWarps, 0, stream>>>(partials, rows, tiles, bn, V1, logits, ld, k, twice,
+                                                                                          stats, top_val, top_idx);
+    CAPB_CHECK_CUDA(cudaGetLastError());
+    return 0;
+}
+
 int ss_select_launch(int rows, int V1, const float* prev_logp, long ld, const long long* labels, long ld_labels, int col, unsigned long long seed, float prob,
                      int* tok_out, cudaStream_t stream) {
     if (rows <= 0) return 0;
diff --git a/include/capb200.h b/include/capb200.h
--- a/include/capb200.h
+++ b/include/capb200.h
@@ -496,6 +496,9 @@
 int capb200_decode_gemm(const float* x, const float* w, int M, int N, int K, int mode, const capb200_gemm_epilogue* epi, unsigned long long* trace_host,
                         int n_slots, void* stream);
 
+int capb200_logit_partials_topk(const float* x, const float* w, const float* bias, int M, int N, int K, int mode, int twice, int k, float* C,
+                                long ldc, float* stats, float* top_val, int* top_idx, void* stream);
+
 #ifdef __cplusplus
 }
 #endif
```

Result: no change. 24150 (median of 6 runs) (+1.0%).
